# mmurooka/SMPLpp

Hardware: NVIDIA B200
Metric: SMPL FK+LBS meshes/s (higher is better)
Workload: dtype f32

## Files before the change

### smplpp_b200/csrc/common.cuh

```cuda
#pragma once
#include <cuda_runtime.h>

#include <atomic>
#include <cstdint>
#include <cstdio>
#include <string>
#include <vector>

#include "../../include/smplpp_b200.h"

namespace sb
{
constexpr int kJoints = SMPLPP_JOINT_NUM;
constexpr int kShapeDim = SMPLPP_SHAPE_DIM;
constexpr int kPoseDim = SMPLPP_POSE_DIM;
constexpr int kBlendK = 224;
constexpr int kBlendKUsed = kPoseDim + kShapeDim + 1;
constexpr int kXformFloats = 12;
constexpr int kGroupVerts = 4;
constexpr int kGroupJoints = 8;

extern thread_local std::string g_last_error;
extern std::atomic<uint64_t> g_launch_count;

int fail(int code, const char * module, const std::string & msg);

#define SB_CUDA(expr)                                                                                   \
  do                                                                                                    \
  {                                                                                                     \
    cudaError_t err__ = (expr);                                                                         \
    if(err__ != cudaSuccess)                                                                            \
      return ::sb::fail(SMPLPP_ERR_CUDA, "CUDA", std::string(#expr) + ": " + cudaGetErrorString(err__)); \
  } while(0)

#define SB_LAUNCHED()                                                              \
  do                                                                               \
  {                                                                                \
    ::sb::g_launch_count.fetch_add(1, std::memory_order_relaxed);                  \
    cudaError_t err__ = cudaPeekAtLastError();                                     \
    if(err__ != cudaSuccess)                                                       \
      return ::sb::fail(SMPLPP_ERR_CUDA, "CUDA", std::string("kernel launch: ") + cudaGetErrorString(err__)); \
  } while(0)

inline cudaStream_t as_stream(void * s)
{
  return static_cast<cudaStream_t>(s);
}

template<typename T>
inline T * align_up_ptr(void * p, size_t a = 256)
{
  return reinterpret_cast<T *>((reinterpret_cast<uintptr_t>(p) + a - 1) / a * a);
}

inline size_t align_up(size_t n, size_t a = 256)
{
  return (n + a - 1) / a * a;
}

inline bool first_call_on_device(bool (&done)[64])
{
  int dev = 0;
  if(cudaGetDevice(&dev) != cudaSuccess || dev < 0 || dev >= 64) return true;
  if(done[dev]) return false;
  done[dev] = true;
  return true;
}

struct ModelDev
{
  int V = 0;
  int Vpad = 0;
  int F = 0;
  int kmax = 0;
  float * basis = nullptr;
  uint8_t * lbs_joint = nullptr;
  float * lbs_weight = nullptr;
  float * lbs_wsum = nullptr;
  int8_t * group_nj = nullptr;
  uint8_t * group_joint = nullptr;
  float * group_w = nullptr;
  float * joint_template = nullptr;
  float * joint_shape = nullptr;
  int parent[kJoints];
  int depth[kJoints];
  int max_depth = 0;
  int32_t * faces = nullptr;
  int32_t * adj_offset = nullptr;
  int32_t * adj_faces = nullptr;
  float * weights_dense = nullptr;
  uint32_t * vert_jmask = nullptr;
  void * basis_split[2] = {nullptr, nullptr};
  alignas(64) unsigned char tmapA[2][128] = {};
  int tc_tiles = 0;
  bool tc_ready = false;
  void * basis_f16 = nullptr;
  alignas(64) unsigned char tmapA16[128] = {};
  int tc2_basis_exp = 0;
  int tc2_tiles = 0;
  bool tc2_ready = false;
  void * basis_img16 = nullptr;
  bool tc3_ready = false;
  int sm_count = 0;
};
}

struct smplpp_model
{
  sb::ModelDev d;
  std::vector<int32_t> h_faces;
  std::vector<int32_t> h_adj_offset;
  std::vector<int32_t> h_adj_faces;
  std::vector<float> h_basis;
  std::vector<float> h_weights;
  std::vector<uint32_t> h_vert_jmask;
  std::vector<float> h_joint_template, h_joint_shape;
  struct HostPipe
  {
    cudaStream_t compute = nullptr, copy = nullptr;
    cudaEvent_t done[2] = {nullptr, nullptr};
    cudaEvent_t drained[2] = {nullptr, nullptr};
    void * dev_in = nullptr;
    size_t dev_in_bytes = 0;
    void * dev_out[2] = {nullptr, nullptr};
    size_t dev_out_bytes = 0;
    void * dev_joints = nullptr;
    size_t dev_joints_bytes = 0;
    void * ws = nullptr;
    size_t ws_bytes = 0;
    void * pin_in = nullptr;
    size_t pin_in_bytes = 0;
    void * pin_out[2] = {nullptr, nullptr};
    size_t pin_out_bytes = 0;
  } pipe;
};
```

### smplpp_b200/csrc/forward.cu

```cuda
#include "common.cuh"
#include "forward.cuh"
#include "ik2.cuh"
#include "ik_poseblend.cuh"
#include "ik_solve.cuh"
#include "tc3_layout.cuh"
#include "vposer.cuh"

using namespace sb;

namespace sb
{
std::atomic<int> g_forward_variant{0};
std::atomic<int> g_lbs_variant{2};
}


__device__ __forceinline__ void rodrigues3(float x, float y, float z, float * R)
{
  const float eps = 1e-8f;
  float ax = x + eps, ay = y + eps, az = z + eps;
  float a = sqrtf(ax * ax + ay * ay + az * az);
  float ux = x / a, uy = y / a, uz = z / a;
  float s, c;
  sincosf(a, &s, &c);
  float oc = 1.f - c;
  R[0] = 1.f + oc * (-(uz * uz) - uy * uy);
  R[1] = s * (-uz) + oc * (uy * ux);
  R[2] = s * uy + oc * (uz * ux);
  R[3] = s * uz + oc * (ux * uy);
  R[4] = 1.f + oc * (-(uz * uz) - ux * ux);
  R[5] = s * (-ux) + oc * (uz * uy);
  R[6] = s * (-uy) + oc * (ux * uz);
  R[7] = s * ux + oc * (uy * uz);
  R[8] = 1.f + oc * (-(uy * uy) - ux * ux);
}

constexpr int kChainWarps = 8;

__global__ void __launch_bounds__(kChainWarps * 32)
    pose_chain_kernel(ChainTopo topo, const float * __restrict__ joint_template,
                      const float * __restrict__ joint_shape, int B, const float * __restrict__ beta,
                      long long beta_stride, const float * __restrict__ theta, float * __restrict__ coef,
                      float * __restrict__ xforms, float * __restrict__ joints_out, float * __restrict__ xforms44_out,
                      uint8_t * __restrict__ img_b, uint8_t * __restrict__ img_g, int Bpad)
{
  __shared__ float sG[kChainWarps][kJoints][12];
  __shared__ float sJ[kChainWarps][kJoints][3];
  __shared__ float sC[kChainWarps][kBlendK];
  const int warp = threadIdx.x >> 5, lane = threadIdx.x & 31;
  const long long b = static_cast<long long>(blockIdx.x) * kChainWarps + warp;
  if(b >= B)
  {
    if(img_b && b < Bpad)
    {
      const long long fb = b / tc3::NF;
      const int nf = static_cast<int>(b - fb * tc3::NF);
      const uint4 z = make_uint4(0u, 0u, 0u, 0u);
      if(lane < tc3::KP / 8)
      {
        uint8_t * blk = img_b + (static_cast<size_t>(fb) * tc3::NKB + lane / 4) * (2 * tc3::B_PART);
        const uint32_t o = static_cast<uint32_t>(tc3::coef_row(nf) * tc3::ROWB + (lane % 4) * 16);
        *reinterpret_cast<uint4 *>(blk + tc3::swz64(o)) = z;
        *reinterpret_cast<uint4 *>(blk + tc3::swz64(tc3::B_PART + o)) = z;
      }
      uint8_t * blk = img_g + (static_cast<size_t>(fb) * tc3::NSUB + nf / tc3::SUBF) * tc3::G_STAGE;
      for(int c = lane; c < kXformFloats * 4; c += 32)
      {
        const uint32_t o = static_cast<uint32_t>(((nf % tc3::SUBF) * kXformFloats + c / 4) * tc3::ROWB + (c % 4) * 16);
        *reinterpret_cast<uint4 *>(blk + tc3::swz64(o)) = z;
        *reinterpret_cast<uint4 *>(blk + tc3::swz64(tc3::G_PART + o)) = z;
      }
    }
    return;
  }

  const float * bp = beta + b * beta_stride;
  float R[9], Jt[3] = {0.f, 0.f, 0.f}, t[3];
  if(lane < kJoints)
  {
    const float * th = theta + (b * (kJoints + 1) + 1 + lane) * 3;
    rodrigues3(th[0], th[1], th[2], R);
#pragma unroll
    for(int k = 0; k < 3; k++)
    {
      float acc = joint_template[lane * 3 + k];
#pragma unroll
      for(int i = 0; i < kShapeDim; i++) acc = fmaf(joint_shape[(lane * 3 + k) * kShapeDim + i], bp[i], acc);
      Jt[k] = acc;
      sJ[warp][lane][k] = acc;
    }
  }
  __syncwarp();
  const int parent = lane < kJoints ? topo.parent[lane] : -1;
  const int depth = lane < kJoints ? topo.depth[lane] : -1;
  if(lane < kJoints)
  {
#pragma unroll
    for(int k = 0; k < 3; k++) t[k] = parent >= 0 ? Jt[k] - sJ[warp][parent][k] : Jt[k];
  }
  float G[12];
  for(int d = 0; d <= topo.max_depth; d++)
  {
    if(depth == d)
    {
      if(parent < 0)
      {
#pragma unroll
        for(int r = 0; r < 3; r++)
        {
          G[4 * r + 0] = R[3 * r + 0];
          G[4 * r + 1] = R[3 * r + 1];
          G[4 * r + 2] = R[3 * r + 2];
          G[4 * r + 3] = t[r];
        }
      }
      else
      {
        const float * P = sG[warp][parent];
#pragma unroll
        for(int r = 0; r < 3; r++)
        {
          float p0 = P[4 * r + 0], p1 = P[4 * r + 1], p2 = P[4 * r + 2], p3 = P[4 * r + 3];
#pragma unroll
          for(int c = 0; c < 3; c++) G[4 * r + c] = p0 * R[c] + p1 * R[3 + c] + p2 * R[6 + c];
          G[4 * r + 3] = p0 * t[0] + p1 * t[1] + p2 * t[2] + p3;
        }
      }
#pragma unroll
      for(int e = 0; e < 12; e++) sG[warp][lane][e] = G[e];
    }
    __syncwarp();
  }
  if(lane < kJoints)
  {
#pragma unroll
    for(int r = 0; r < 3; r++) G[4 * r + 3] -= G[4 * r + 0] * Jt[0] + G[4 * r + 1] * Jt[1] + G[4 * r + 2] * Jt[2];
    if(xforms)
    {
      float4 * dst = reinterpret_cast<float4 *>(xforms + (b * kJoints + lane) * 12);
      dst[0] = make_float4(G[0], G[1], G[2], G[3]);
      dst[1] = make_float4(G[4], G[5], G[6], G[7]);
      dst[2] = make_float4(G[8], G[9], G[10], G[11]);
    }
    if(xforms44_out)
    {
      float4 * dst = reinterpret_cast<float4 *>(xforms44_out + (b * kJoints + lane) * 16);
      dst[0] = make_float4(G[0], G[1], G[2], G[3]);
      dst[1] = make_float4(G[4], G[5], G[6], G[7]);
      dst[2] = make_float4(G[8], G[9], G[10], G[11]);
      dst[3] = make_float4(0.f, 0.f, 0.f, 1.f);
    }
    if(joints_out)
    {
#pragma unroll
      for(int k = 0; k < 3; k++) joints_out[(b * kJoints + lane) * 3 + k] = Jt[k];
    }
  }
  if(img_g)
  {
    __syncwarp();
    if(lane < kJoints)
    {
#pragma unroll
      for(int e = 0; e < 12; e++) sG[warp][lane][e] = G[e];
    }
    __syncwarp();
    const long long fb = b / tc3::NF;
    const int nf = static_cast<int>(b - fb * tc3::NF);
    uint8_t * blk = img_g + (static_cast<size_t>(fb) * tc3::NSUB + nf / tc3::SUBF) * tc3::G_STAGE;
    for(int c = lane; c < kXformFloats * 4; c += 32)
    {
      const int e = c / 4, cj = c % 4;
      float x[8];
#pragma unroll
      for(int jj = 0; jj < 8; jj++)
      {
        const int j = cj * 8 + jj;
        x[jj] = j < kJoints ? sG[warp][j][e] * static_cast<float>(1 << tc3::G_EXP) : 0.f;
      }
      const uint32_t o = static_cast<uint32_t>(((nf % tc3::SUBF) * kXformFloats + e) * tc3::ROWB + cj * 16);
      tc3::split8_store(x, blk + tc3::swz64(o), blk + tc3::swz64(tc3::G_PART + o));
    }
  }
  if(coef)
  {
    if(lane >= 1 && lane < kJoints)
    {
#pragma unroll
      for(int e = 0; e < 9; e++) sC[warp][9 * (lane - 1) + e] = R[e] - ((e == 0 || e == 4 || e == 8) ? 1.f : 0.f);
    }
    if(lane < kShapeDim) sC[warp][kPoseDim + lane] = bp[lane];
    if(lane >= kShapeDim && lane < kShapeDim + 1 + (kBlendK - kBlendKUsed))
      sC[warp][kPoseDim + lane] = lane == kShapeDim ? 1.f : 0.f;
    __syncwarp();
    for(int i = lane; i < kBlendK; i += 32) coef[b * kBlendK + i] = sC[warp][i];
    if(img_b && lane < tc3::KP / 8)
    {
      float x[8];
#pragma unroll
      for(int e = 0; e < 8; e++) x[e] = lane * 8 + e < tc3::KUSED ? sC[warp][lane * 8 + e] * static_cast<float>(1 << tc3::COEF_EXP) : 0.f;
      const long long fb = b / tc3::NF;
      const int r = tc3::coef_row(static_cast<int>(b - fb * tc3::NF));
      uint8_t * blk = img_b + (static_cast<size_t>(fb) * tc3::NKB + lane / 4) * (2 * tc3::B_PART);
      const uint32_t o = static_cast<uint32_t>(r * tc3::ROWB + (lane % 4) * 16);
      tc3::split8_store(x, blk + tc3::swz64(o), blk + tc3::swz64(tc3::B_PART + o));
    }
  }
}

namespace k2
{
constexpr int BM = 64, BNV = 64, BN = BNV * 3, BK = 16, THREADS = 256;
constexpr int TM = 4, TNV = 4, TN = TNV * 3;
constexpr int AS_LD = BM + 4, BS_LD = BN + 4;
constexpr int GS_LD = kJoints * 12;
constexpr size_t SMEM_AB = sizeof(float) * 2 * BK * (AS_LD + BS_LD);
constexpr size_t SMEM_G = sizeof(float) * BM * GS_LD;
constexpr size_t SMEM_TOTAL = SMEM_AB + SMEM_G;
}

__device__ __forceinline__ void cp_async16(void * smem, const void * gmem)
{
  unsigned s = static_cast<unsigned>(__cvta_generic_to_shared(smem));
  asm volatile("cp.async.cg.shared.global [%0], [%1], 16;\n" ::"r"(s), "l"(gmem));
}
__device__ __forceinline__ void cp_async_commit()
{
  asm volatile("cp.async.commit_group;\n" ::);
}
__device__ __forceinline__ void cp_async_wait_all()
{
  asm volatile("cp.async.wait_all;\n" ::);
}

template<bool kSkin>
__global__ void __launch_bounds__(k2::THREADS, 2)
    blend_skin_ffma_kernel(const float * __restrict__ basis, const uint8_t * __restrict__ lbs_joint,
                           const float * __restrict__ lbs_weight, const float * __restrict__ lbs_wsum, int V, int Vpad,
                           int kmax, int B, const float * __restrict__ coef, const float * __restrict__ xforms,
                           const float * __restrict__ theta, float * __restrict__ out)
{
  using namespace k2;
  extern __shared__ __align__(16) float smem[];
  float * As = smem;
  float * Bs = smem + 2 * BK * AS_LD;
  float * Gs = smem + 2 * BK * (AS_LD + BS_LD);

  const int tid = threadIdx.x;
  const int tx = tid & 15, ty = tid >> 4;
  const int v0 = blockIdx.x * BNV;
  const int m0 = blockIdx.y * BM;

  if(kSkin)
  {
    for(int i = tid; i < BM * GS_LD / 4; i += THREADS)
    {
      int row = i / (GS_LD / 4), q = i % (GS_LD / 4);
      int b = min(m0 + row, B - 1);
      cp_async16(Gs + row * GS_LD + q * 4, xforms + static_cast<size_t>(b) * GS_LD + q * 4);
    }
    cp_async_commit();
  }

  const int a_row = tid >> 2, a_q = tid & 3;
  const float * a_src = coef + static_cast<size_t>(min(m0 + a_row, B - 1)) * kBlendK + a_q * 4;
  const float * b_src[3];
  int b_row[3], b_q[3];
#pragma unroll
  for(int i = 0; i < 3; i++)
  {
    int idx = tid + i * THREADS;
    b_row[i] = idx >> 2;
    b_q[i] = idx & 3;
    b_src[i] = basis + (static_cast<size_t>(v0) * 3 + b_row[i]) * kBlendK + b_q[i] * 4;
  }
  float4 a_reg, b_reg[3];
  auto load_chunk = [&](int kc) {
    a_reg = __ldg(reinterpret_cast<const float4 *>(a_src + kc * BK));
#pragma unroll
    for(int i = 0; i < 3; i++) b_reg[i] = __ldg(reinterpret_cast<const float4 *>(b_src[i] + kc * BK));
  };
  auto store_chunk = [&](int buf) {
    float * as = As + buf * BK * AS_LD + (a_q * 4) * AS_LD + a_row;
    as[0] = a_reg.x;
    as[AS_LD] = a_reg.y;
    as[2 * AS_LD] = a_reg.z;
    as[3 * AS_LD] = a_reg.w;
#pragma unroll
    for(int i = 0; i < 3; i++)
    {
      float * bs = Bs + buf * BK * BS_LD + (b_q[i] * 4) * BS_LD + b_row[i];
      bs[0] = b_reg[i].x;
      bs[BS_LD] = b_reg[i].y;
      bs[2 * BS_LD] = b_reg[i].z;
      bs[3 * BS_LD] = b_reg[i].w;
    }
  };

  float acc[TM][TN];
#pragma unroll
  for(int i = 0; i < TM; i++)
#pragma unroll
    for(int j = 0; j < TN; j++) acc[i][j] = 0.f;

  constexpr int NK = kBlendK / BK;
  load_chunk(0);
  store_chunk(0);
  __syncthreads();
  for(int kc = 0; kc < NK; kc++)
  {
    const int buf = kc & 1;
    if(kc + 1 < NK) load_chunk(kc + 1);
    const float * as = As + buf * BK * AS_LD + ty * TM;
    const float * bs = Bs + buf * BK * BS_LD + tx * TN;
#pragma unroll
    for(int k = 0; k < BK; k++)
    {
      float4 a4 = *reinterpret_cast<const float4 *>(as + k * AS_LD);
      float4 b0 = *reinterpret_cast<const float4 *>(bs + k * BS_LD);
      float4 b1 = *reinterpret_cast<const float4 *>(bs + k * BS_LD + 4);
      float4 b2 = *reinterpret_cast<const float4 *>(bs + k * BS_LD + 8);
      float a[TM] = {a4.x, a4.y, a4.z, a4.w};
      float bb[TN] = {b0.x, b0.y, b0.z, b0.w, b1.x, b1.y, b1.z, b1.w, b2.x, b2.y, b2.z, b2.w};
#pragma unroll
      for(int i = 0; i < TM; i++)
#pragma unroll
        for(int j = 0; j < TN; j++) acc[i][j] = fmaf(a[i], bb[j], acc[i][j]);
    }
    if(kc + 1 < NK)
    {
      store_chunk(buf ^ 1);
      __syncthreads();
    }
  }

  const int vbase = v0 + tx * TNV;
  const bool vec_ok = (V & 1) == 0;
  if(kSkin)
  {
    cp_async_wait_all();
    __syncthreads();
    uint8_t jn[TNV][4];
    float jw[TNV][4], inv_ws[TNV];
    if(kmax <= 4)
    {
#pragma unroll
      for(int jv = 0; jv < TNV; jv++)
      {
#pragma unroll
        for(int k = 0; k < 4; k++)
        {
          bool on = k < kmax;
          jn[jv][k] = on ? lbs_joint[static_cast<size_t>(k) * Vpad + vbase + jv] : 0;
          jw[jv][k] = on ? lbs_weight[static_cast<size_t>(k) * Vpad + vbase + jv] : 0.f;
        }
        inv_ws[jv] = 1.f / lbs_wsum[vbase + jv];
      }
    }
#pragma unroll
    for(int i = 0; i < TM; i++)
    {
      const int b = m0 + ty * TM + i;
      if(b >= B) continue;
      const float * g = Gs + (ty * TM + i) * GS_LD;
      const float * tr = theta + static_cast<size_t>(b) * (kJoints + 1) * 3;
      const float trx = tr[0], try_ = tr[1], trz = tr[2];
      float o[TN];
#pragma unroll
      for(int jv = 0; jv < TNV; jv++)
      {
        const float rx = acc[i][3 * jv], ry = acc[i][3 * jv + 1], rz = acc[i][3 * jv + 2];
        float ox = 0.f, oy = 0.f, oz = 0.f, iw;
        if(kmax <= 4)
        {
#pragma unroll
          for(int k = 0; k < 4; k++)
          {
            const float4 * gj = reinterpret_cast<const float4 *>(g + jn[jv][k] * 12);
            float4 r0 = gj[0], r1 = gj[1], r2 = gj[2];
            float w = jw[jv][k];
            ox = fmaf(w, fmaf(r0.x, rx, fmaf(r0.y, ry, fmaf(r0.z, rz, r0.w))), ox);
            oy = fmaf(w, fmaf(r1.x, rx, fmaf(r1.y, ry, fmaf(r1.z, rz, r1.w))), oy);
            oz = fmaf(w, fmaf(r2.x, rx, fmaf(r2.y, ry, fmaf(r2.z, rz, r2.w))), oz);
          }
          iw = inv_ws[jv];
        }
        else
        {
          const int v = vbase + jv;
          for(int k = 0; k < kmax; k++)
          {
            const float4 * gj = reinterpret_cast<const float4 *>(g + lbs_joint[static_cast<size_t>(k) * Vpad + v] * 12);
            float4 r0 = gj[0], r1 = gj[1], r2 = gj[2];
            float w = lbs_weight[static_cast<size_t>(k) * Vpad + v];
            ox = fmaf(w, fmaf(r0.x, rx, fmaf(r0.y, ry, fmaf(r0.z, rz, r0.w))), ox);
            oy = fmaf(w, fmaf(r1.x, rx, fmaf(r1.y, ry, fmaf(r1.z, rz, r1.w))), oy);
            oz = fmaf(w, fmaf(r2.x, rx, fmaf(r2.y, ry, fmaf(r2.z, rz, r2.w))), oz);
          }
          iw = 1.f / lbs_wsum[v];
        }
        o[3 * jv] = fmaf(ox, iw, trx);
        o[3 * jv + 1] = fmaf(oy, iw, try_);
        o[3 * jv + 2] = fmaf(oz, iw, trz);
      }
      float * dst = out + (static_cast<size_t>(b) * V + vbase) * 3;
      if(vbase + TNV <= V && vec_ok)
      {
#pragma unroll
        for(int q = 0; q < TN / 2; q++) reinterpret_cast<float2 *>(dst)[q] = make_float2(o[2 * q], o[2 * q + 1]);
      }
      else
      {
        for(int q = 0; q < TN; q++)
          if(vbase + q / 3 < V) dst[q] = o[q];
      }
    }
  }
  else
  {
#pragma unroll
    for(int i = 0; i < TM; i++)
    {
      const int b = m0 + ty * TM + i;
      if(b >= B) continue;
      float * dst = out + (static_cast<size_t>(b) * V + vbase) * 3;
      if(vbase + TNV <= V && vec_ok)
      {
#pragma unroll
        for(int q = 0; q < TN / 2; q++) reinterpret_cast<float2 *>(dst)[q] = make_float2(acc[i][2 * q], acc[i][2 * q + 1]);
      }
      else
      {
        for(int q = 0; q < TN; q++)
          if(vbase + q / 3 < V) dst[q] = acc[i][q];
      }
    }
  }
}

namespace k3
{
constexpr int THREADS = 256, VPL = kGroupVerts, VPC = THREADS * VPL;
constexpr int FR = 16;
}

template<bool kAffine, bool kVec2>
__global__ void __launch_bounds__(k3::THREADS, 2)
    lbs_kernel(const uint8_t * __restrict__ lbs_joint, const float * __restrict__ lbs_weight,
               const float * __restrict__ lbs_wsum, const int8_t * __restrict__ group_nj,
               const uint8_t * __restrict__ group_joint, const float * __restrict__ group_w, int V, int Vpad, int kmax,
               int B, const float * __restrict__ rest, const float * __restrict__ xforms,
               const float * __restrict__ root, int root_stride, float * __restrict__ out)
{
  using namespace k3;
  constexpr int XF = kAffine ? 12 : 16;
  constexpr int XFP = kAffine ? 12 : 20;
  __shared__ __align__(16) float Gs[FR][kJoints * XFP];
  const int tid = threadIdx.x;
  const int b0 = blockIdx.y * FR;
  const int nfr = min(FR, B - b0);
  for(int i = tid; i < nfr * kJoints * XF / 4; i += THREADS)
  {
    const int fr = i / (kJoints * XF / 4), rem = i % (kJoints * XF / 4);
    const int j = rem / (XF / 4), q = rem % (XF / 4);
    *reinterpret_cast<float4 *>(&Gs[fr][j * XFP + 4 * q]) =
        __ldg(reinterpret_cast<const float4 *>(xforms + static_cast<size_t>(b0) * kJoints * XF) + i);
  }
  const int v = (blockIdx.x * THREADS + tid) * VPL;
  const int g = v / VPL;
  const int nvalid = min(VPL, V - v);
  int nj = -1;
  float gw[kGroupJoints][VPL], iw[VPL];
  unsigned gj_lo = 0, gj_hi = 0;
  if(nvalid > 0)
  {
    nj = group_nj ? group_nj[g] : -1;
#pragma unroll
    for(int u = 0; u < VPL; u++) iw[u] = 1.f / lbs_wsum[min(v + u, V - 1)];
    if(nj >= 0)
    {
      const uint2 jj = __ldg(reinterpret_cast<const uint2 *>(group_joint + static_cast<size_t>(g) * kGroupJoints));
      gj_lo = jj.x, gj_hi = jj.y;
#pragma unroll
      for(int k = 0; k < kGroupJoints; k++)
      {
        const float4 w = __ldg(reinterpret_cast<const float4 *>(group_w + (static_cast<size_t>(g) * kGroupJoints + k) * VPL));
        gw[k][0] = w.x, gw[k][1] = w.y, gw[k][2] = w.z, gw[k][3] = w.w;
      }
    }
  }
  __syncthreads();
  if(nvalid <= 0) return;
  const bool full = nvalid == VPL;
  float rn[3 * VPL];
  auto load_frame = [&](int f) {
    const size_t base = (static_cast<size_t>(b0 + f) * V + v) * 3;
    if(kVec2 && full)
    {
      const float2 * src = reinterpret_cast<const float2 *>(rest + base);
#pragma unroll
      for(int q = 0; q < 6; q++)
      {
        const float2 t = __ldcs(src + q);
        rn[2 * q] = t.x, rn[2 * q + 1] = t.y;
      }
    }
    else
    {
#pragma unroll
      for(int q = 0; q < 3 * VPL; q++) rn[q] = q < 3 * nvalid ? rest[base + q] : 0.f;
    }
  };
  load_frame(0);
  for(int f = 0; f < nfr; f++)
  {
    const size_t base = (static_cast<size_t>(b0 + f) * V + v) * 3;
    float r[3 * VPL];
#pragma unroll
    for(int q = 0; q < 3 * VPL; q++) r[q] = rn[q];
    if(f + 1 < nfr) load_frame(f + 1);
    float tx = 0.f, ty = 0.f, tz = 0.f;
    if(root)
    {
      const float * rp = root + static_cast<size_t>(b0 + f) * root_stride;
      tx = rp[0], ty = rp[1], tz = rp[2];
    }
    float o[3 * VPL], ow[VPL];
#pragma unroll
    for(int q = 0; q < 3 * VPL; q++) o[q] = 0.f;
#pragma unroll
    for(int u = 0; u < VPL; u++) ow[u] = 0.f;
    if(nj >= 0)
    {
#pragma unroll
      for(int k = 0; k < kGroupJoints; k++)
      {
        if(k < nj)
        {
          const int j = ((k < 4 ? gj_lo : gj_hi) >> (8 * (k & 3))) & 0xff;
          const float4 * gjp = reinterpret_cast<const float4 *>(&Gs[f][j * XFP]);
          const float4 r0 = gjp[0], r1 = gjp[1], r2 = gjp[2];
          float4 r3 = make_float4(0.f, 0.f, 0.f, 1.f);
          if(!kAffine) r3 = gjp[3];
#pragma unroll
          for(int u = 0; u < VPL; u++)
          {
            const float w = gw[k][u];
            const float rx = r[3 * u], ry = r[3 * u + 1], rz = r[3 * u + 2];
            o[3 * u] = fmaf(w, fmaf(r0.x, rx, fmaf(r0.y, ry, fmaf(r0.z, rz, r0.w))), o[3 * u]);
            o[3 * u + 1] = fmaf(w, fmaf(r1.x, rx, fmaf(r1.y, ry, fmaf(r1.z, rz, r1.w))), o[3 * u + 1]);
            o[3 * u + 2] = fmaf(w, fmaf(r2.x, rx, fmaf(r2.y, ry, fmaf(r2.z, rz, r2.w))), o[3 * u + 2]);
            if(!kAffine) ow[u] = fmaf(w, fmaf(r3.x, rx, fmaf(r3.y, ry, fmaf(r3.z, rz, r3.w))), ow[u]);
          }
        }
      }
    }
    else
    {
      for(int u = 0; u < nvalid; u++)
      {
        const float rx = r[3 * u], ry = r[3 * u + 1], rz = r[3 * u + 2];
        float ox = 0.f, oy = 0.f, oz = 0.f, o4 = 0.f;
        for(int k = 0; k < kmax; k++)
        {
          const float w = lbs_weight[static_cast<size_t>(k) * Vpad + v + u];
          const float4 * gjp = reinterpret_cast<const float4 *>(&Gs[f][lbs_joint[static_cast<size_t>(k) * Vpad + v + u] * XFP]);
          const float4 r0 = gjp[0], r1 = gjp[1], r2 = gjp[2];
          ox = fmaf(w, fmaf(r0.x, rx, fmaf(r0.y, ry, fmaf(r0.z, rz, r0.w))), ox);
          oy = fmaf(w, fmaf(r1.x, rx, fmaf(r1.y, ry, fmaf(r1.z, rz, r1.w))), oy);
          oz = fmaf(w, fmaf(r2.x, rx, fmaf(r2.y, ry, fmaf(r2.z, rz, r2.w))), oz);
          if(!kAffine)
          {
            const float4 r3 = gjp[3];
            o4 = fmaf(w, fmaf(r3.x, rx, fmaf(r3.y, ry, fmaf(r3.z, rz, r3.w))), o4);
          }
        }
#pragma unroll
        for(int uu = 0; uu < VPL; uu++)
          if(uu == u) o[3 * uu] = ox, o[3 * uu + 1] = oy, o[3 * uu + 2] = oz, ow[uu] = o4;
      }
    }
#pragma unroll
    for(int u = 0; u < VPL; u++)
    {
      const float inv = kAffine ? iw[u] : 1.f / ow[u];
      o[3 * u] = fmaf(o[3 * u], inv, tx);
      o[3 * u + 1] = fmaf(o[3 * u + 1], inv, ty);
      o[3 * u + 2] = fmaf(o[3 * u + 2], inv, tz);
    }
    if(kVec2 && full)
    {
      float2 * dst = reinterpret_cast<float2 *>(out + base);
#pragma unroll
      for(int q = 0; q < 6; q++) __stcs(dst + q, make_float2(o[2 * q], o[2 * q + 1]));
    }
    else
    {
#pragma unroll
      for(int q = 0; q < 3 * VPL; q++)
        if(q < 3 * nvalid) out[base + q] = o[q];
    }
  }
}

__global__ void rodrigues_kernel(long long n, const float * __restrict__ theta, float * __restrict__ rot)
{
  long long i = static_cast<long long>(blockIdx.x) * blockDim.x + threadIdx.x;
  if(i >= n) return;
  float R[9];
  rodrigues3(theta[3 * i], theta[3 * i + 1], theta[3 * i + 2], R);
#pragma unroll
  for(int e = 0; e < 9; e++) rot[9 * i + e] = R[e];
}

__global__ void blend_generic_kernel(int B, int V, const float * __restrict__ beta, const float * __restrict__ rot,
                                     const float * __restrict__ shape_basis, const float * __restrict__ pose_basis,
                                     float * __restrict__ shape_bs, float * __restrict__ pose_bs)
{
  long long i = static_cast<long long>(blockIdx.x) * blockDim.x + threadIdx.x;
  if(i >= static_cast<long long>(B) * V * 3) return;
  int b = static_cast<int>(i / (static_cast<long long>(V) * 3));
  long long vk = i % (static_cast<long long>(V) * 3);
  const float * pb = pose_basis + vk * kPoseDim;
  const float * r = rot + static_cast<size_t>(b) * kJoints * 9 + 9;
  float acc = 0.f;
  for(int d = 0; d < kPoseDim; d++)
  {
    int e = d % 9;
    float c = r[d] - ((e == 0 || e == 4 || e == 8) ? 1.f : 0.f);
    acc = fmaf(c, pb[d], acc);
  }
  pose_bs[i] = acc;
  const float * sb_ = shape_basis + vk * kShapeDim;
  float s = 0.f;
  for(int d = 0; d < kShapeDim; d++) s = fmaf(beta[b * kShapeDim + d], sb_[d], s);
  shape_bs[i] = s;
}

__global__ void linear_combine_kernel(long long n, long long vk_count, const float * __restrict__ templ,
                                      const float * __restrict__ shape_bs, const float * __restrict__ pose_bs,
                                      float * __restrict__ rest)
{
  long long i = static_cast<long long>(blockIdx.x) * blockDim.x + threadIdx.x;
  if(i >= n) return;
  rest[i] = templ[i % vk_count] + shape_bs[i] + pose_bs[i];
}

__global__ void joint_regress_kernel(int B, int V, const float * __restrict__ templ, const float * __restrict__ jreg,
                                     const float * __restrict__ shape_bs, float * __restrict__ joints)
{
  int w = (blockIdx.x * blockDim.x + threadIdx.x) >> 5, lane = threadIdx.x & 31;
  if(w >= B * kJoints * 3) return;
  int b = w / (kJoints * 3), j = (w / 3) % kJoints, k = w % 3;
  float acc = 0.f;
  for(int v = lane; v < V; v += 32)
    acc = fmaf(jreg[static_cast<size_t>(j) * V + v], templ[3 * v + k] + shape_bs[(static_cast<size_t>(b) * V + v) * 3 + k], acc);
#pragma unroll
  for(int o = 16; o > 0; o >>= 1) acc += __shfl_xor_sync(0xffffffffu, acc, o);
  if(lane == 0) joints[w] = acc;
}

__global__ void world_transform_kernel(int B, const long long * __restrict__ kine_tree, const float * __restrict__ joints,
                                       const float * __restrict__ rot, float * __restrict__ out)
{
  int b = blockIdx.x * blockDim.x + threadIdx.x;
  if(b >= B) return;
  float G[kJoints][12];
  const float * J = joints + static_cast<size_t>(b) * kJoints * 3;
  const float * R = rot + static_cast<size_t>(b) * kJoints * 9;
  for(int j = 0; j < kJoints; j++)
  {
    long long p = kine_tree[j];
    const float * Rj = R + 9 * j;
    if(j == 0 || p < 0 || p >= kJoints)
    {
      for(int r = 0; r < 3; r++)
      {
        for(int c = 0; c < 3; c++) G[j][4 * r + c] = Rj[3 * r + c];
        G[j][4 * r + 3] = J[3 * j + r];
      }
    }
    else
    {
      float t[3] = {J[3 * j] - J[3 * p], J[3 * j + 1] - J[3 * p + 1], J[3 * j + 2] - J[3 * p + 2]};
      for(int r = 0; r < 3; r++)
      {
        float p0 = G[p][4 * r], p1 = G[p][4 * r + 1], p2 = G[p][4 * r + 2], p3 = G[p][4 * r + 3];
        for(int c = 0; c < 3; c++) G[j][4 * r + c] = p0 * Rj[c] + p1 * Rj[3 + c] + p2 * Rj[6 + c];
        G[j][4 * r + 3] = p0 * t[0] + p1 * t[1] + p2 * t[2] + p3;
      }
    }
  }
  float * o = out + static_cast<size_t>(b) * kJoints * 16;
  for(int j = 0; j < kJoints; j++)
  {
    for(int r = 0; r < 3; r++)
    {
      for(int c = 0; c < 3; c++) o[16 * j + 4 * r + c] = G[j][4 * r + c];
      o[16 * j + 4 * r + 3] =
          G[j][4 * r + 3] - (G[j][4 * r] * J[3 * j] + G[j][4 * r + 1] * J[3 * j + 1] + G[j][4 * r + 2] * J[3 * j + 2]);
    }
    o[16 * j + 12] = 0.f, o[16 * j + 13] = 0.f, o[16 * j + 14] = 0.f, o[16 * j + 15] = 1.f;
  }
}

__global__ void lbs_dense_kernel(int B, int V, const float * __restrict__ weights, const float * __restrict__ rest,
                                 const float * __restrict__ xf, const float * __restrict__ root,
                                 float * __restrict__ out)
{
  long long i = static_cast<long long>(blockIdx.x) * blockDim.x + threadIdx.x;
  if(i >= static_cast<long long>(B) * V) return;
  int b = static_cast<int>(i / V), v = static_cast<int>(i % V);
  float rx = rest[3 * i], ry = rest[3 * i + 1], rz = rest[3 * i + 2];
  float M[16];
  for(int e = 0; e < 16; e++) M[e] = 0.f;
  for(int j = 0; j < kJoints; j++)
  {
    float w = weights[static_cast<size_t>(v) * kJoints + j];
    const float * g = xf + (static_cast<size_t>(b) * kJoints + j) * 16;
    for(int e = 0; e < 16; e++) M[e] = fmaf(w, g[e], M[e]);
  }
  float h[4];
  for(int r = 0; r < 4; r++) h[r] = M[4 * r] * rx + M[4 * r + 1] * ry + M[4 * r + 2] * rz + M[4 * r + 3];
  for(int k = 0; k < 3; k++) out[3 * i + k] = h[k] / h[3] + (root ? root[3 * b + k] : 0.f);
}

__device__ __forceinline__ void normalize3(float & x, float & y, float & z)
{
  float n = fmaxf(sqrtf(x * x + y * y + z * z), 1e-12f);
  x /= n, y /= n, z /= n;
}

__device__ __forceinline__ void face_normal(const float * __restrict__ verts, const int32_t * __restrict__ faces, int f,
                                            float & nx, float & ny, float & nz)
{
  const float * a = verts + 3 * faces[3 * f], *b = verts + 3 * faces[3 * f + 1], *c = verts + 3 * faces[3 * f + 2];
  float e1x = b[0] - a[0], e1y = b[1] - a[1], e1z = b[2] - a[2];
  float e2x = c[0] - a[0], e2y = c[1] - a[1], e2z = c[2] - a[2];
  nx = e1y * e2z - e1z * e2y;
  ny = e1z * e2x - e1x * e2z;
  nz = e1x * e2y - e1y * e2x;
  normalize3(nx, ny, nz);
}

__global__ void normals_kernel(const int32_t * __restrict__ faces, const int32_t * __restrict__ adj_offset,
                               const int32_t * __restrict__ adj_faces, int V, int F, int B,
                               const float * __restrict__ verts, int nF, const long long * __restrict__ face_idx,
                               float * __restrict__ fn, int nV, const long long * __restrict__ vert_idx,
                               float * __restrict__ vn)
{
  long long i = static_cast<long long>(blockIdx.x) * blockDim.x + threadIdx.x;
  const int per = nF + nV;
  if(i >= static_cast<long long>(B) * per) return;
  int b = static_cast<int>(i / per), it = static_cast<int>(i % per);
  const float * vb = verts + static_cast<size_t>(b) * V * 3;
  if(it < nF)
  {
    long long f = face_idx[it];
    float x = 0.f, y = 0.f, z = 0.f;
    if(f >= 0 && f < F) face_normal(vb, faces, static_cast<int>(f), x, y, z);
    float * o = fn + (static_cast<size_t>(b) * nF + it) * 3;
    o[0] = x, o[1] = y, o[2] = z;
  }
  else
  {
    it -= nF;
    long long v = vert_idx[it];
    float ax = 0.f, ay = 0.f, az = 0.f;
    if(v >= 0 && v < V)
    {
      int s = adj_offset[v], e = adj_offset[v + 1];
      float w = 1.f / static_cast<float>(e - s);
      for(int k = s; k < e; k++)
      {
        float x, y, z;
        face_normal(vb, faces, adj_faces[k], x, y, z);
        ax = fmaf(w, x, ax), ay = fmaf(w, y, ay), az = fmaf(w, z, az);
      }
      normalize3(ax, ay, az);
    }
    float * o = vn + (static_cast<size_t>(b) * nV + it) * 3;
    o[0] = ax, o[1] = ay, o[2] = az;
  }
}

namespace sb
{
ChainTopo make_topo(const ModelDev & d)
{
  ChainTopo t;
  for(int j = 0; j < kJoints; j++)
  {
    t.parent[j] = d.parent[j];
    t.depth[j] = d.depth[j];
  }
  t.max_depth = d.max_depth;
  return t;
}

int launch_pose_chain(const ModelDev & d, cudaStream_t st, int B, const float * beta, long long beta_stride,
                      const float * theta, float * coef, float * xforms, float * joints, float * xforms44,
                      void * tc3_scratch)
{
  const int Bpad = tc3_scratch ? static_cast<int>(align_up(static_cast<size_t>(B), tc3::NF)) : B;
  uint8_t * img_b = static_cast<uint8_t *>(tc3_scratch);
  uint8_t * img_g = tc3_scratch ? img_b + tc3::img_g_offset(Bpad) : nullptr;
  int grid = (Bpad + kChainWarps - 1) / kChainWarps;
  pose_chain_kernel<<<grid, kChainWarps * 32, 0, st>>>(make_topo(d), d.joint_template, d.joint_shape, B, beta,
                                                       beta_stride, theta, coef, xforms, joints, xforms44, img_b, img_g, Bpad);
  SB_LAUNCHED();
  return SMPLPP_OK;
}

int launch_blend_skin_ffma(const ModelDev & d, cudaStream_t st, int B, const float * coef, const float * xforms,
                           const float * theta, float * out, bool skin)
{
  static bool configured[64] = {};
  if(first_call_on_device(configured))
  {
    SB_CUDA(cudaFuncSetAttribute(blend_skin_ffma_kernel<true>, cudaFuncAttributeMaxDynamicSharedMemorySize,
                                 static_cast<int>(k2::SMEM_TOTAL)));
    SB_CUDA(cudaFuncSetAttribute(blend_skin_ffma_kernel<false>, cudaFuncAttributeMaxDynamicSharedMemorySize,
                                 static_cast<int>(k2::SMEM_AB)));
  }
  dim3 grid(d.Vpad / k2::BNV, (B + k2::BM - 1) / k2::BM);
  if(skin)
    blend_skin_ffma_kernel<true><<<grid, k2::THREADS, k2::SMEM_TOTAL, st>>>(
        d.basis, d.lbs_joint, d.lbs_weight, d.lbs_wsum, d.V, d.Vpad, d.kmax, B, coef, xforms, theta, out);
  else
    blend_skin_ffma_kernel<false><<<grid, k2::THREADS, k2::SMEM_AB, st>>>(
        d.basis, d.lbs_joint, d.lbs_weight, d.lbs_wsum, d.V, d.Vpad, d.kmax, B, coef, xforms, theta, out);
  SB_LAUNCHED();
  return SMPLPP_OK;
}

int launch_lbs(const ModelDev & d, cudaStream_t st, int B, const float * rest, const float * xforms, bool affine,
               const float * root, int root_stride, float * out)
{
  if(affine && g_lbs_variant == 2 && lbs_tc_usable(d, rest, out, xforms))
    return launch_lbs_tc(d, st, B, rest, xforms, kXformFloats, root, root_stride, out);
  if(affine && g_lbs_variant == 0 && lbs_tma_usable(d, rest, out, xforms))
    return launch_lbs_tma(d, st, B, rest, xforms, root, root_stride, out);
  dim3 grid((d.V + k3::VPC - 1) / k3::VPC, (B + k3::FR - 1) / k3::FR);
  const bool vec2 = (d.V & 1) == 0 && (reinterpret_cast<uintptr_t>(rest) & 7) == 0 && (reinterpret_cast<uintptr_t>(out) & 7) == 0;
#define SB_LBS(AFF, VEC)                                                                                               \
  lbs_kernel<AFF, VEC><<<grid, k3::THREADS, 0, st>>>(d.lbs_joint, d.lbs_weight, d.lbs_wsum, d.group_nj, d.group_joint, \
                                                     d.group_w, d.V, d.Vpad, d.kmax, B, rest, xforms, root,           \
                                                     root_stride, out)
  if(affine && vec2)
    SB_LBS(true, true);
  else if(affine)
    SB_LBS(true, false);
  else if(vec2)
    SB_LBS(false, true);
  else
    SB_LBS(false, false);
#undef SB_LBS
  SB_LAUNCHED();
  return SMPLPP_OK;
}
}

extern "C" int smplpp_set_forward_variant(int variant)
{
  if(variant == 100 || variant == 101)
  {
    g_tc_grid_order = variant - 100;
    return SMPLPP_OK;
  }
  if(variant == 300 || variant == 301)
  {
    g_vposer_jac_variant = variant - 300;
    return SMPLPP_OK;
  }
  if(variant >= 200 && variant <= 202)
  {
    g_lbs_variant = variant - 200;
    return SMPLPP_OK;
  }
  if(variant >= 400 && variant <= 402)
  {
    g_ik_variant = variant - 400;
    return SMPLPP_OK;
  }
  if(variant == 410 || variant == 411)
  {
    g_solve_variant = variant - 410;
    return SMPLPP_OK;
  }
  if(variant >= 420 && variant <= 422)
  {
    g_poseblend_variant = variant - 420;
    return SMPLPP_OK;
  }
  if(variant < 0 || variant > 6) return fail(SMPLPP_ERR_INVALID, "SMPL", "unknown forward variant");
  g_forward_variant = variant;
  return SMPLPP_OK;
}

extern "C" size_t smplpp_forward_workspace_bytes(const smplpp_model_t * model, int64_t batch)
{
  if(!model || batch < 1) return 0;
  size_t bpad = align_up(static_cast<size_t>(batch), 128);
  size_t bytes = 512;
  bytes += align_up(bpad * kBlendK * sizeof(float));
  bytes += align_up(bpad * kJoints * 12 * sizeof(float));
  bytes += tc_coef_split_bytes(batch);
  bytes += std::max(tc2_frame_operand_bytes(batch), tc3_frame_operand_bytes(batch));
  bytes += align_up(static_cast<size_t>(batch) * model->d.V * 3 * sizeof(float));
  return bytes;
}

extern "C" int smplpp_forward(const smplpp_model_t * model, void * stream, int64_t batch, const float * beta,
                              int64_t beta_stride, const float * theta, float * vertices, float * joints,
                              float * transforms, float * rest_shape, void * workspace, size_t workspace_bytes)
{
  if(!model || batch < 1 || !beta || !theta) return fail(SMPLPP_ERR_INVALID, "SMPL", "Cannot launch a SMPL model!");
  if(batch > (1ll << 24)) return fail(SMPLPP_ERR_INVALID, "SMPL", "Cannot launch a SMPL model! (batch too large)");
  if(!workspace || workspace_bytes < smplpp_forward_workspace_bytes(model, batch))
    return fail(SMPLPP_ERR_INVALID, "SMPL", "Cannot launch a SMPL model! (workspace too small)");
  const ModelDev & d = model->d;
  const int B = static_cast<int>(batch);
  cudaStream_t st = as_stream(stream);
  size_t bpad = align_up(static_cast<size_t>(batch), 128);
  char * ws = align_up_ptr<char>(workspace);
  float * coef = reinterpret_cast<float *>(ws);
  ws += align_up(bpad * kBlendK * sizeof(float));
  float * xforms = reinterpret_cast<float *>(ws);
  ws += align_up(bpad * kJoints * 12 * sizeof(float));
  void * coef_split = ws;
  ws += tc_coef_split_bytes(batch);
  void * tc2_scratch = ws;
  ws += std::max(tc2_frame_operand_bytes(batch), tc3_frame_operand_bytes(batch));
  float * rest_ws = reinterpret_cast<float *>(ws);

  const bool need_verts = vertices != nullptr;
  const bool need_rest = rest_shape != nullptr;
  int variant = g_forward_variant;
  if(variant == 0) variant = model->d.tc3_ready ? 6 : (model->d.tc2_ready ? 5 : (model->d.tc_ready ? 2 : 1));
  if(((variant == 2 || variant == 4) && !model->d.tc_ready) || (variant == 5 && !model->d.tc2_ready)
     || (variant == 6 && !model->d.tc3_ready))
    return fail(SMPLPP_ERR_INVALID, "SMPL", "tcgen05 blend variant is not available for this model");
  const bool fused_images = variant == 6 && need_verts && !need_rest;
  int rc = launch_pose_chain(d, st, B, beta, beta_stride, theta, (need_verts || need_rest) ? coef : nullptr, xforms,
                             joints, transforms, fused_images ? tc2_scratch : nullptr);
  if(rc != SMPLPP_OK) return rc;
  if(need_rest || (need_verts && variant == 3))
  {
    float * rest = need_rest ? rest_shape : rest_ws;
    rc = launch_blend_skin_ffma(d, st, B, coef, xforms, theta, rest, false);
    if(rc != SMPLPP_OK) return rc;
    if(need_verts) rc = launch_lbs(d, st, B, rest, xforms, true, theta, (kJoints + 1) * 3, vertices);
    return rc;
  }
  if(need_verts)
  {
    if(variant == 6)
      rc = launch_blend_skin_tc3(d, st, B, coef, xforms, tc2_scratch, theta, vertices, true);
    else if(variant == 5)
      rc = launch_blend_skin_tc2(d, st, B, coef, xforms, tc2_scratch, theta, vertices);
    else if(variant == 2 || variant == 4)
      rc = launch_blend_skin_tc(d, st, B, coef, coef_split, xforms, theta, vertices, variant == 2);
    else
      rc = launch_blend_skin_ffma(d, st, B, coef, xforms, theta, vertices, true);
  }
  return rc;
}


extern "C" int smplpp_blend_shape(void * stream, int64_t batch, int64_t V, const float * beta, const float * theta,
                                  const float * shape_basis, const float * pose_basis, float * shape_bs, float * pose_bs,
                                  float * pose_rot)
{
  if(batch < 1 || V < 1 || !beta) return fail(SMPLPP_ERR_INVALID, "BlendShape", "Failed to set beta!");
  if(!theta) return fail(SMPLPP_ERR_INVALID, "BlendShape", "Failed to set theta!");
  if(!shape_basis || !pose_basis || !shape_bs || !pose_bs || !pose_rot)
    return fail(SMPLPP_ERR_INVALID, "BlendShape", "Cannot blend pose-dependented shape!");
  cudaStream_t st = as_stream(stream);
  long long n = batch * kJoints;
  rodrigues_kernel<<<static_cast<unsigned>((n + 127) / 128), 128, 0, st>>>(n, theta, pose_rot);
  SB_LAUNCHED();
  long long total = batch * V * 3;
  blend_generic_kernel<<<static_cast<unsigned>((total + 127) / 128), 128, 0, st>>>(
      static_cast<int>(batch), static_cast<int>(V), beta, pose_rot, shape_basis, pose_basis, shape_bs, pose_bs);
  SB_LAUNCHED();
  return SMPLPP_OK;
}

extern "C" int smplpp_joint_regression(void * stream, int64_t batch, int64_t V, const float * templ, const float * jreg,
                                       const float * shape_bs, const float * pose_bs, float * rest, float * joints)
{
  if(batch < 1 || V < 1 || !templ || !shape_bs || !pose_bs || !rest)
    return fail(SMPLPP_ERR_INVALID, "JointRegression", "Cannot linearly combine shapes!");
  if(!jreg || !joints) return fail(SMPLPP_ERR_INVALID, "JointRegression", "Cannot regress vertices to joints!");
  cudaStream_t st = as_stream(stream);
  long long n = batch * V * 3;
  linear_combine_kernel<<<static_cast<unsigned>((n + 255) / 256), 256, 0, st>>>(n, V * 3, templ, shape_bs, pose_bs, rest);
  SB_LAUNCHED();
  long long warps = batch * kJoints * 3;
  joint_regress_kernel<<<static_cast<unsigned>((warps * 32 + 127) / 128), 128, 0, st>>>(
      static_cast<int>(batch), static_cast<int>(V), templ, jreg, shape_bs, joints);
  SB_LAUNCHED();
  return SMPLPP_OK;
}

extern "C" int smplpp_world_transformation(void * stream, int64_t batch, const int64_t * kine_tree, const float * joints,
                                           const float * pose_rot, float * transforms)
{
  if(batch < 1 || !kine_tree || !joints || !pose_rot || !transforms)
    return fail(SMPLPP_ERR_INVALID, "WorldTransformation", "Cannot transform bones locally!");
  world_transform_kernel<<<static_cast<unsigned>((batch + 63) / 64), 64, 0, as_stream(stream)>>>(
      static_cast<int>(batch), reinterpret_cast<const long long *>(kine_tree), joints, pose_rot, transforms);
  SB_LAUNCHED();
  return SMPLPP_OK;
}

extern "C" int smplpp_linear_blend_skinning(void * stream, int64_t batch, int64_t V, const float * weights,
                                            const float * rest, const float * transforms, const float * root_pos,
                                            float * vertices)
{
  if(batch < 1 || V < 1 || !weights) return fail(SMPLPP_ERR_INVALID, "LinearBlendSkinning", "Failed to set weights!");
  if(!rest || !transforms || !vertices)
    return fail(SMPLPP_ERR_INVALID, "LinearBlendSkinning", "Cannot convert Cartesian coordinates to homogeneous one!");
  long long n = batch * V;
  lbs_dense_kernel<<<static_cast<unsigned>((n + 127) / 128), 128, 0, as_stream(stream)>>>(
      static_cast<int>(batch), static_cast<int>(V), weights, rest, transforms, root_pos, vertices);
  SB_LAUNCHED();
  return SMPLPP_OK;
}

extern "C" int smplpp_model_skinning(const smplpp_model_t * model, void * stream, int64_t batch, const float * rest,
                                     const float * transforms, const float * root_pos, float * vertices)
{
  if(!model || batch < 1 || !rest || !transforms || !vertices)
    return fail(SMPLPP_ERR_INVALID, "LinearBlendSkinning", "Failed to get vertices of new pose!");
  return launch_lbs(model->d, as_stream(stream), static_cast<int>(batch), rest, transforms, false, root_pos, 3, vertices);
}

extern "C" int smplpp_normals(const smplpp_model_t * model, void * stream, int64_t batch, const float * vertices,
                              int64_t n_faces, const int64_t * face_idx, float * face_normals, int64_t n_verts,
                              const int64_t * vert_idx, float * vertex_normals)
{
  if(!model || batch < 1 || !vertices || n_faces < 0 || n_verts < 0 || (n_faces > 0 && (!face_idx || !face_normals))
     || (n_verts > 0 && (!vert_idx || !vertex_normals)))
    return fail(SMPLPP_ERR_INVALID, "SMPL", "Failed to get face indices!");
  long long total = batch * (n_faces + n_verts);
  if(total == 0) return SMPLPP_OK;
  const ModelDev & d = model->d;
  normals_kernel<<<static_cast<unsigned>((total + 127) / 128), 128, 0, as_stream(stream)>>>(
      d.faces, d.adj_offset, d.adj_faces, d.V, d.F, static_cast<int>(batch), vertices, static_cast<int>(n_faces),
      reinterpret_cast<const long long *>(face_idx), face_normals, static_cast<int>(n_verts),
      reinterpret_cast<const long long *>(vert_idx), vertex_normals);
  SB_LAUNCHED();
  return SMPLPP_OK;
}

extern "C" int smplpp_model_skinning34(const smplpp_model_t * model, void * stream, int64_t batch, const float * rest,
                                       const float * transforms34, const float * root_pos, float * vertices)
{
  if(!model || batch < 1 || !rest || !transforms34 || !vertices)
    return fail(SMPLPP_ERR_INVALID, "LinearBlendSkinning", "Failed to get vertices of new pose!");
  return launch_lbs(model->d, as_stream(stream), static_cast<int>(batch), rest, transforms34, true, root_pos, 3, vertices);
}
```

### smplpp_b200/csrc/skin_tc3.cu

```cuda
#include <cuda.h>
#include <cuda_fp16.h>

#include <cstdio>
#include <cstdlib>
#include <vector>

#include "forward.cuh"
#include "skin_common.cuh"
#include "tc3_layout.cuh"
#include "tc_ptx.cuh"

using namespace sb;

namespace tc3
{
struct Params
{
  int V, B, Bpad, ntiles, nfb, nitems;
  float scale_p, scale_m;
  const uint8_t * img_a;
  const uint8_t * img_b;
  const uint8_t * img_g;
  const float * basis;
  const float * weights;
  const float * wsum;
  const float * theta;
  float * out;
  long long * dbg;
  int dbg_mode;
};

}

__global__ void basis_image_f16_kernel(const float * __restrict__ basis, int V, int ntiles, float scale, uint8_t * __restrict__ img)
{
  const long long i = static_cast<long long>(blockIdx.x) * blockDim.x + threadIdx.x;
  const long long n = static_cast<long long>(ntiles) * 3 * tc3::MV * tc3::KP;
  if(i >= n) return;
  const int k = static_cast<int>(i % tc3::KP);
  const long long row = i / tc3::KP;
  const int r = static_cast<int>(row % tc3::MV);
  const int plane = static_cast<int>((row / tc3::MV) % 3);
  const int tile = static_cast<int>(row / (3 * tc3::MV));
  const int v = tile * tc3::MV + r;
  const float x = (v < V && k < tc3::KUSED) ? basis[(static_cast<size_t>(3) * v + plane) * kBlendK + k] * scale : 0.f;
  const __half hi = __float2half_rn(x);
  const __half lo = __float2half_rn(x - __half2float(hi));
  uint8_t * blk = img + (static_cast<size_t>(tile) * tc3::NKB + k / 32) * (2 * tc3::A_PART);
  const uint32_t o = static_cast<uint32_t>(plane * tc3::MV * tc3::ROWB + r * tc3::ROWB + (k % 32) * 2);
  *reinterpret_cast<__half *>(blk + tc3::swz64(o)) = hi;
  *reinterpret_cast<__half *>(blk + tc3::swz64(tc3::A_PART + o)) = lo;
}

__global__ void frame_images3_kernel(const float * __restrict__ coef, const float * __restrict__ xforms, int B, int Bpad,
                                     uint8_t * __restrict__ img_b, uint8_t * __restrict__ img_g)
{
  const long long i = static_cast<long long>(blockIdx.x) * blockDim.x + threadIdx.x;
  constexpr int CK = tc3::KP / 8;
  constexpr int CJ = tc3::KJ / 8;
  const long long n_coef = static_cast<long long>(Bpad) * CK;
  const long long n_xf = static_cast<long long>(Bpad) * kXformFloats * CJ;
  float x[8];
  if(i < n_coef)
  {
    const int ck = static_cast<int>(i % CK);
    const long long f = i / CK;
    if(f < B)
    {
      const float4 a = __ldg(reinterpret_cast<const float4 *>(coef + f * tc3::KP + ck * 8));
      const float4 b = __ldg(reinterpret_cast<const float4 *>(coef + f * tc3::KP + ck * 8 + 4));
      x[0] = a.x, x[1] = a.y, x[2] = a.z, x[3] = a.w, x[4] = b.x, x[5] = b.y, x[6] = b.z, x[7] = b.w;
    }
#pragma unroll
    for(int e = 0; e < 8; e++) x[e] = (f < B && ck * 8 + e < tc3::KUSED) ? x[e] * static_cast<float>(1 << tc3::COEF_EXP) : 0.f;
    const long long fb = f / tc3::NF;
    const int r = tc3::coef_row(static_cast<int>(f - fb * tc3::NF));
    uint8_t * blk = img_b + (static_cast<size_t>(fb) * tc3::NKB + ck / 4) * (2 * tc3::B_PART);
    const uint32_t o = static_cast<uint32_t>(r * tc3::ROWB + (ck % 4) * 16);
    tc3::split8_store(x, blk + tc3::swz64(o), blk + tc3::swz64(tc3::B_PART + o));
  }
  else if(i < n_coef + n_xf)
  {
    const long long q = i - n_coef;
    const int cj = static_cast<int>(q % CJ);
    const long long row = q / CJ;
    const int e = static_cast<int>(row % kXformFloats);
    const long long f = row / kXformFloats;
#pragma unroll
    for(int jj = 0; jj < 8; jj++)
    {
      const int j = cj * 8 + jj;
      x[jj] = (f < B && j < kJoints) ? __ldg(xforms + (f * kJoints + j) * kXformFloats + e) * static_cast<float>(1 << tc3::G_EXP) : 0.f;
    }
    const long long fb = f / tc3::NF;
    const int nf = static_cast<int>(f - fb * tc3::NF);
    uint8_t * blk = img_g + (static_cast<size_t>(fb) * tc3::NSUB + nf / tc3::SUBF) * tc3::G_STAGE;
    const uint32_t o = static_cast<uint32_t>(((nf % tc3::SUBF) * kXformFloats + e) * tc3::ROWB + cj * 16);
    tc3::split8_store(x, blk + tc3::swz64(o), blk + tc3::swz64(tc3::G_PART + o));
  }
}

template<int STAGES, int GSLOTS, int EPI, bool DBG = false>
__global__ void __launch_bounds__(tc3::THREADS, 1)
    blend_skin_tc3_kernel(const tc3::Params p)
{
  using namespace tc3;
  using L = Layout<STAGES, GSLOTS, EPI>;
  constexpr int OFF_G = L::OFF_G, OFF_STG = L::OFF_STG, OFF_BAR = L::OFF_BAR;
  extern __shared__ uint8_t smem_raw[];
  uint8_t * smem = reinterpret_cast<uint8_t *>((reinterpret_cast<uintptr_t>(smem_raw) + 1023) & ~uintptr_t(1023));
  uint64_t * bars = reinterpret_cast<uint64_t *>(smem + OFF_BAR);
  const uint32_t smem32 = (ptx::smem_u32(smem_raw) + 1023u) & ~1023u;
  const uint32_t bar32 = smem32 + OFF_BAR;
  uint64_t * full = bars;
  uint64_t * empty = full + STAGES;
  uint64_t * g_full = empty + STAGES;
  uint64_t * g_empty = g_full + GSLOTS;
  uint64_t * m_full = g_empty + GSLOTS;
  uint64_t * m_empty = m_full + 2;
  uint64_t * p_full = m_empty + 2;
  uint64_t * rest_free = p_full + 1;
  uint64_t * w_ready = rest_free + 1;
  uint32_t * tmem_slot = reinterpret_cast<uint32_t *>(w_ready + 1);

  const int warp = threadIdx.x >> 5, lane = threadIdx.x & 31;
  const int it0 = static_cast<int>(static_cast<long long>(blockIdx.x) * p.nitems / gridDim.x);
  const int it1 = static_cast<int>(static_cast<long long>(blockIdx.x + 1) * p.nitems / gridDim.x);
  const int nit = it1 - it0;

  if(warp == 0 && lane == 0)
  {
    for(int s = 0; s < STAGES; s++)
    {
      ptx::mbar_init(&full[s], 1);
      ptx::mbar_init(&empty[s], 1);
    }
    for(int s = 0; s < GSLOTS; s++)
    {
      ptx::mbar_init(&g_full[s], 1);
      ptx::mbar_init(&g_empty[s], 1);
    }
    for(int i = 0; i < 2; i++)
    {
      ptx::mbar_init(&m_full[i], 1);
      ptx::mbar_init(&m_empty[i], EPI_WARPS);
    }
    ptx::mbar_init(p_full, 1);
    ptx::mbar_init(rest_free, EPI_WARPS);
    ptx::mbar_init(w_ready, 4);
    ptx::fence_barrier_init();
  }
  if(warp == 1) ptx::tmem_alloc<TMEM_COLS>(tmem_slot);
  ptx::tc_fence_before();
  __syncthreads();
  ptx::tc_fence_after();
  const uint32_t tmem_base = *tmem_slot;
  long long * dbg = (DBG && p.dbg) ? p.dbg + static_cast<size_t>(blockIdx.x) * 256 : nullptr;
  long long w_stage = 0, w_gfull = 0, w_mempty = 0, w_rest = 0, w_pfull = 0, w_mfull = 0;
#define TC3_OFF(bit) (DBG && (p.dbg_mode & (bit)))
#define TC3_TIMED(acc, stmt) do { if constexpr(DBG) { const long long t_ = clock64(); stmt; acc += clock64() - t_; } else { stmt; } } while(0)

  if(warp < CTRL_WARPS)
  {
  asm volatile("setmaxnreg.dec.sync.aligned.u32 32;");
  if(warp == 0)
  {
    if(ptx::elect_one())
    {
      const int total_kb = TC3_OFF(32) ? 0 : nit * NKB;
      int kb = 0, tile = it0 / p.nfb, fb = it0 % p.nfb;
      for(int kbn = 0; kbn < total_kb; kbn++)
      {
        const uint32_t s = static_cast<uint32_t>(kbn % STAGES);
        const uint8_t * srca = p.img_a + (static_cast<size_t>(tile) * NKB + kb) * (2 * A_PART);
        const uint8_t * srcb = p.img_b + (static_cast<size_t>(fb) * NKB + kb) * (2 * B_PART);
        const uint32_t dst = smem32 + s * STAGE, fbar = bar32 + 8 * s;
        ptx::mbar_wait_a(bar32 + 8 * (STAGES + s), ((kbn / STAGES) & 1) ^ 1);
        ptx::mbar_expect_tx_a(fbar, STAGE);
        ptx::bulk_load_1d_a(dst, srca, 2 * A_PART, fbar);
        ptx::bulk_load_1d_a(dst + 2 * A_PART, srcb, 2 * B_PART, fbar);
        if(dbg && kbn < 14) dbg[34 + kbn] = clock64();
        if(++kb == NKB)
        {
          kb = 0;
          if(++fb == p.nfb) fb = 0, tile++;
        }
      }
    }
  }
  else if(warp == 2)
  {
    if(ptx::elect_one())
    {
      const int total_g = TC3_OFF(64) ? 0 : nit * NSUB;
      int sb = 0, fb = it0 % p.nfb;
      for(int gn = 0; gn < total_g; gn++)
      {
        const uint32_t s = static_cast<uint32_t>(gn % GSLOTS);
        const uint8_t * src = p.img_g + (static_cast<size_t>(fb) * NSUB + sb) * G_STAGE;
        const uint32_t fbar = bar32 + 8 * (2 * STAGES + s);
        ptx::mbar_wait_a(bar32 + 8 * (2 * STAGES + GSLOTS + s), ((gn / GSLOTS) & 1) ^ 1);
        ptx::mbar_expect_tx_a(fbar, G_STAGE);
        ptx::bulk_load_1d_a(smem32 + OFF_G + s * G_STAGE, src, G_STAGE, fbar);
        if(++sb == NSUB)
        {
          sb = 0;
          if(++fb == p.nfb) fb = 0;
        }
      }
    }
  }
  else if(warp == 1 || warp == 3)
  {
    if(ptx::elect_one())
    {
      constexpr uint32_t idesc1 = ptx::make_idesc_f16(MV, NF);
      constexpr uint32_t idesc2 = ptx::make_idesc_f16(MV, SUBN);
      static_assert(NSUB % GSLOTS == 0 && ((NSUB / GSLOTS) & 1) == 0, "transform ring: slot and parity of a sub-batch do not depend on the item");
      static_assert((NSUB & 3) == 0, "matrix buffers: parity of a sub-batch does not depend on the item");
      constexpr uint32_t DHI = ptx::smem_desc_hi<ROWB>();
      const uint32_t smem16 = smem32 >> 4;
      const uint32_t a_full = bar32;
      const uint32_t a_empty = a_full + 8 * STAGES, a_gfull = a_empty + 8 * STAGES, a_gempty = a_gfull + 8 * GSLOTS,
                     a_mfull = a_gempty + 8 * GSLOTS, a_mempty = a_mfull + 16, a_pfull = a_mempty + 16, a_rest = a_pfull + 8,
                     a_wready = a_rest + 8;
      auto g1_mma = [&](uint32_t st16, int hpar, int i, uint32_t acc) {
        const int t = i / 3, c = i % 3;
        const int a_part = hpar == 0 ? (t == 2 ? 1 : 0) : (t == 0 ? 1 : 0);
        const int b_part = hpar == 0 ? 0 : (t == 0 ? 0 : 1);
        const int ks = hpar == 0 ? (t == 1 ? 1 : 0) : (t == 1 ? 0 : 1);
        ptx::umma_f16_ss_lo(tmem_base + c * NF, st16 + ((a_part * A_PART + c * MV * ROWB + ks * 32) >> 4),
                            st16 + ((2 * A_PART + b_part * B_PART + ks * 32) >> 4), DHI, idesc1, acc);
      };
      auto g2_mma = [&](uint32_t dm, uint32_t aw, uint32_t sg16, int j) {
        const int prod = j >> 1, ks = j & 1;
        const int pa = prod == 1 ? 1 : 0, pb = prod == 2 ? 1 : 0;
        ptx::umma_f16_ts_lo(dm, aw + pa * (KJ / 2) + ks * 8, sg16 + ((pb * G_PART + ks * 32) >> 4), DHI, idesc2, j != 0 ? 1u : 0u);
      };
      auto g1_half = [&](int h, int kbn0) {
        const int kbn = kbn0 + (h >> 1);
        const uint32_t s = static_cast<uint32_t>(kbn % STAGES);
        const uint32_t st16 = smem16 + s * (STAGE >> 4);
        if((h & 1) == 0)
        {
          if(!TC3_OFF(32)) TC3_TIMED(w_stage, ptx::mbar_wait_a(a_full + 8 * s, (kbn / STAGES) & 1));
          ptx::tc_fence_after();
          if(dbg && kbn < 14) dbg[48 + kbn] = clock64();
#pragma unroll
          for(int i = 0; i < 9; i++)
            if(!DBG || !(p.dbg_mode & 8)) g1_mma(st16, 0, i, (h == 0 && i < 3) ? 0u : 1u);
        }
        else
        {
#pragma unroll
          for(int i = 0; i < 9; i++)
            if(!DBG || !(p.dbg_mode & 8)) g1_mma(st16, 1, i, 1u);
          if(!TC3_OFF(32)) ptx::tc_commit_a(a_empty + 8 * s);
        }
      };
      if(dbg) dbg[0] = clock64();
      if(nit > 0 && warp == 3)
      {
#pragma unroll
        for(int h = 0; h < 2 * NKB; h++) g1_half(h, 0);
        if(!TC3_OFF(512)) ptx::tc_commit_a(a_pfull);
      }
      if(dbg) dbg[1] = clock64();
      if(warp == 3)
      {
        for(int k = 0; k + 1 < nit; k++)
        {
          if(!TC3_OFF(512)) TC3_TIMED(w_rest, ptx::mbar_wait_a(a_rest, k & 1));
          ptx::tc_fence_after();
#pragma unroll
          for(int h = 0; h < 2 * NKB; h++) g1_half(h, (k + 1) * NKB);
          if(!TC3_OFF(512)) ptx::tc_commit_a(a_pfull);
        }
        if(dbg) dbg[64] = w_stage, dbg[67] = w_rest, dbg[69] = clock64();
      }
      int wcount = 0, prev_tile = -1;
      for(int k = 0; k < (warp == 3 ? 0 : nit); k++)
      {
        const int tile = (it0 + k) / p.nfb;
        if(tile != prev_tile)
        {
          ptx::mbar_wait_a(a_wready, wcount & 1);
          ptx::tc_fence_after();
          wcount++;
          prev_tile = tile;
        }
        const uint32_t aw = tmem_base + COL_W;
#pragma unroll
        for(int sb = 0; sb < NSUB; sb++)
        {
          const int b = sb & 1, gs = sb % GSLOTS;
          if(!TC3_OFF(64)) TC3_TIMED(w_gfull, ptx::mbar_wait_a(a_gfull + 8 * gs, (sb / GSLOTS) & 1));
          if(!TC3_OFF(256)) TC3_TIMED(w_mempty, ptx::mbar_wait_a(a_mempty + 8 * b, ((sb >> 1) & 1) ^ 1));
          ptx::tc_fence_after();
          const uint32_t sg16 = smem16 + ((OFF_G + gs * G_STAGE) >> 4);
          const uint32_t dm = tmem_base + COL_M + b * SUBN;
#pragma unroll
          for(int j = 0; j < 6; j++)
            if(!DBG || !(p.dbg_mode & 4)) g2_mma(dm, aw, sg16, j);
          if(!TC3_OFF(256)) ptx::tc_commit_a(a_mfull + 8 * b);
          if(!TC3_OFF(64)) ptx::tc_commit_a(a_gempty + 8 * gs);
        }
        if(dbg && k < 30) dbg[2 + k] = clock64();
      }
      if(dbg && warp == 1) dbg[65] = w_gfull, dbg[66] = w_mempty, dbg[68] = clock64();
    }
  }
  }
  else
  {
    asm volatile("setmaxnreg.inc.sync.aligned.u32 112;");
    const int ew = warp - CTRL_WARPS;
    const int q = warp & 3;
    const int fp = ew >> 2;
    const uint32_t lane_taddr = tmem_base + (static_cast<uint32_t>(q * 32) << 16);
    const uint32_t my_stg = ptx::smem_u32(smem + OFF_STG) + ew * STG_FLOATS * 4;
    const float sp = p.scale_p;
    const uint32_t a_mfull = bar32 + 16 * (STAGES + GSLOTS);
    const uint32_t a_mempty = a_mfull + 16, a_pfull = a_mempty + 16, a_rest = a_pfull + 8, a_wready = a_rest + 8;
    const unsigned fstride = static_cast<unsigned>(p.V) * 3u;
    int prev_tile = -1;
    int wv0 = 0, nvalid = 0;
    float T0 = 0.f, T1 = 0.f, T2 = 0.f, sm = 0.f;
    if(dbg && ew == 0 && lane == 0) dbg[32] = clock64();
    for(int k = 0; k < nit; k++)
    {
      const int item = it0 + k;
      const int tile = item / p.nfb, f0 = (item - tile * p.nfb) * NF;
      if(tile != prev_tile)
      {
        prev_tile = tile;
        wv0 = tile * MV + q * 32;
        const int vc = min(wv0 + lane, p.V - 1);
        nvalid = max(0, min(32, p.V - wv0));
        if(ew < 4)
        {
          skin::store_w_row_tmem(p.weights + static_cast<size_t>(vc) * kJoints, lane_taddr + COL_W);
          ptx::tmem_st_wait();
          ptx::tc_fence_before();
          __syncwarp();
          if(lane == 0) ptx::mbar_arrive_a(a_wready);
        }
        sm = p.scale_m / p.wsum[vc];
        const float * tp = p.basis + static_cast<size_t>(3) * vc * kBlendK + KUSED;
        T0 = __ldg(tp) * sm, T1 = __ldg(tp + kBlendK) * sm, T2 = __ldg(tp + 2 * kBlendK) * sm;
      }
      float trx = 0.f, try_ = 0.f, trz = 0.f;
      if(lane < FR_WARP)
      {
        const int f = min(f0 + (lane >> 1) * SUBF + fp * EPI_FR + (lane & 1), p.B - 1);
        const float * tq = p.theta + static_cast<size_t>(f) * ((kJoints + 1) * 3);
        trx = __ldg(tq), try_ = __ldg(tq + 1), trz = __ldg(tq + 2);
      }
      float R[3][FR_WARP];
      if(!TC3_OFF(512)) TC3_TIMED(w_pfull, ptx::mbar_wait_a(a_pfull, k & 1));
      ptx::tc_fence_after();
#pragma unroll
      for(int c = 0; c < 3; c++)
      {
        if(DBG && (p.dbg_mode & 16))
        {
#pragma unroll
          for(int i = 0; i < FR_WARP; i++) R[c][i] = 1.f;
          continue;
        }
        ptx::tmem_ld_x16(lane_taddr + c * NF + fp * FR_WARP, R[c]);
        ptx::tmem_ld_x8p(lane_taddr + c * NF + fp * FR_WARP + 16, R[c] + 16);
      }
      ptx::tmem_ld_wait();
      ptx::tc_fence_before();
      __syncwarp();
      if(lane == 0 && !TC3_OFF(512)) ptx::mbar_arrive_a(a_rest);
      {
        const float s = sp * sm;
#pragma unroll
        for(int i = 0; i < FR_WARP; i++)
        {
          R[0][i] = fmaf(R[0][i], s, T0);
          R[1][i] = fmaf(R[1][i], s, T1);
          R[2][i] = fmaf(R[2][i], s, T2);
        }
      }
      float * outp = p.out + (static_cast<size_t>(f0 + fp * EPI_FR) * p.V + wv0) * 3;
      float * outl = outp + lane * 3;
      const int nfv = lane < nvalid ? p.B - f0 - fp * EPI_FR : 0;
#pragma unroll
      for(int sb = 0; sb < NSUB; sb++)
      {
        const int h = sb & 1;
        float tr[EPI_FR][3];
#pragma unroll
        for(int t = 0; t < EPI_FR; t++)
        {
          tr[t][0] = __shfl_sync(0xffffffffu, trx, sb * EPI_FR + t);
          tr[t][1] = __shfl_sync(0xffffffffu, try_, sb * EPI_FR + t);
          tr[t][2] = __shfl_sync(0xffffffffu, trz, sb * EPI_FR + t);
        }
        if(!TC3_OFF(256)) TC3_TIMED(w_mfull, ptx::mbar_wait_a(a_mfull + 8 * h, (sb >> 1) & 1));
        ptx::tc_fence_after();
        float M[EPI_FR * kXformFloats];
        const uint32_t mcol = lane_taddr + COL_M + h * SUBN + fp * (EPI_FR * kXformFloats);
        if(DBG && (p.dbg_mode & 1))
        {
#pragma unroll
          for(int i = 0; i < EPI_FR * kXformFloats; i++) M[i] = 1.f + i;
        }
        else
        {
          ptx::tmem_ld_x16(mcol, M);
          ptx::tmem_ld_x8p(mcol + 16, M + 16);
        }
        ptx::tmem_ld_wait();
        ptx::tc_fence_before();
        __syncwarp();
        if(lane == 0 && !TC3_OFF(256)) ptx::mbar_arrive_a(a_mempty + 8 * h);
        if(TC3_OFF(128)) continue;
#pragma unroll
        for(int t = 0; t < EPI_FR; t++)
        {
          const float rx = R[0][sb * EPI_FR + t], ry = R[1][sb * EPI_FR + t], rz = R[2][sb * EPI_FR + t];
          const float * m = M + kXformFloats * t;
          const float ox = fmaf(m[0], rx, fmaf(m[1], ry, fmaf(m[2], rz, fmaf(m[3], sm, tr[t][0]))));
          const float oy = fmaf(m[4], rx, fmaf(m[5], ry, fmaf(m[6], rz, fmaf(m[7], sm, tr[t][1]))));
          const float oz = fmaf(m[8], rx, fmaf(m[9], ry, fmaf(m[10], rz, fmaf(m[11], sm, tr[t][2]))));
          if constexpr(EPI == 0)
          {
            const uint32_t sa = my_stg + (t * 96 + lane * 3) * 4;
            ptx::sts32(sa, ox);
            ptx::sts32(sa + 4, oy);
            ptx::sts32(sa + 8, oz);
          }
          else
          {
            float * o = outl + static_cast<size_t>((sb * SUBF + t) * fstride);
            if(sb * SUBF + t < nfv && (!DBG || !(p.dbg_mode & 2) || ox == 1.2345e30f))
            {
              __stcs(o, ox);
              __stcs(o + 1, oy);
              __stcs(o + 2, oz);
            }
          }
        }
        if constexpr(EPI != 0) continue;
        __syncwarp();
#pragma unroll
        for(int i = 0; i < EPI_FR * 48 / 32; i++)
        {
          const int idx = 32 * i + lane;
          const int t = idx / 48;
          const int w2 = idx - 48 * t;
          const int f = f0 + sb * SUBF + fp * EPI_FR + t;
          const float2 val = ptx::lds64(my_stg + idx * 8);
          if(f < p.B && 2 * w2 < 3 * nvalid)
            __stcs(reinterpret_cast<float2 *>(outp + (static_cast<size_t>(sb * SUBF + t) * p.V) * 3) + w2, val);
        }
        __syncwarp();
      }
    }
    if(dbg && (ew == 0 || ew == 15) && lane == 0)
    {
      if(ew == 0) dbg[33] = clock64();
      dbg[70 + (ew ? 2 : 0)] = w_pfull, dbg[71 + (ew ? 2 : 0)] = w_mfull;
    }
  }
#undef TC3_TIMED
#undef TC3_OFF
  ptx::tc_fence_before();
  __syncthreads();
  if(warp == 1) ptx::tmem_dealloc<TMEM_COLS>(tmem_base);
}

namespace sb
{
size_t tc3_frame_operand_bytes(int64_t batch)
{
  const size_t bpad = align_up(static_cast<size_t>(batch), tc3::NF);
  return align_up(2 * bpad * tc3::KP * sizeof(__half)) + align_up(2 * bpad * kXformFloats * tc3::KJ * sizeof(__half));
}

int tc3_prepare_model(ModelDev & d)
{
  d.tc3_ready = false;
  if(!d.tc2_ready) return SMPLPP_OK;
  const long long n = static_cast<long long>(d.tc2_tiles) * 3 * tc3::MV * tc3::KP;
  SB_CUDA(cudaMalloc(&d.basis_img16, static_cast<size_t>(2) * n * sizeof(__half)));
  basis_image_f16_kernel<<<static_cast<unsigned>((n + 255) / 256), 256>>>(d.basis, d.V, d.tc2_tiles, ldexpf(1.f, d.tc2_basis_exp),
                                                                         static_cast<uint8_t *>(d.basis_img16));
  SB_LAUNCHED();
  SB_CUDA(cudaDeviceSynchronize());
  SB_CUDA(cudaFuncSetAttribute(blend_skin_tc3_kernel<2, 6, 1>, cudaFuncAttributeMaxDynamicSharedMemorySize, tc3::Layout<2, 6, 1>::SMEM_BYTES));
  SB_CUDA(cudaFuncSetAttribute(blend_skin_tc3_kernel<2, 6, 1, true>, cudaFuncAttributeMaxDynamicSharedMemorySize, tc3::Layout<2, 6, 1>::SMEM_BYTES));
  SB_CUDA(cudaFuncSetAttribute(blend_skin_tc3_kernel<3, 3, 1>, cudaFuncAttributeMaxDynamicSharedMemorySize, tc3::Layout<3, 3, 1>::SMEM_BYTES));
  SB_CUDA(cudaFuncSetAttribute(blend_skin_tc3_kernel<2, 6, 0>, cudaFuncAttributeMaxDynamicSharedMemorySize, tc3::Layout<2, 6, 0>::SMEM_BYTES));
  int dev = 0;
  SB_CUDA(cudaGetDevice(&dev));
  SB_CUDA(cudaDeviceGetAttribute(&d.sm_count, cudaDevAttrMultiProcessorCount, dev));
  d.tc3_ready = d.sm_count > 0;
  return SMPLPP_OK;
}

void tc3_release_model(ModelDev & d)
{
  if(d.basis_img16) cudaFree(d.basis_img16);
  d.basis_img16 = nullptr;
  d.tc3_ready = false;
}

int launch_blend_skin_tc3(const ModelDev & d, cudaStream_t st, int B, const float * coef, const float * xforms, void * scratch,
                          const float * theta, float * out, bool images_ready)
{
  if(!d.tc3_ready) return fail(SMPLPP_ERR_INVALID, "SMPL", "pipelined tcgen05 skinning variant is not available for this model");
  if(reinterpret_cast<uintptr_t>(out) & 7) return fail(SMPLPP_ERR_INVALID, "SMPL", "tcgen05 variants need 8-byte aligned vertices");
  if(reinterpret_cast<uintptr_t>(scratch) & 127) return fail(SMPLPP_ERR_INVALID, "SMPL", "tcgen05 variants need a 128-byte aligned workspace");
  const int Bpad = static_cast<int>(align_up(static_cast<size_t>(B), tc3::NF));
  uint8_t * img_b = static_cast<uint8_t *>(scratch);
  uint8_t * img_g = img_b + tc3::img_g_offset(Bpad);
  if(!images_ready)
  {
    const long long n = static_cast<long long>(Bpad) * (tc3::KP + kXformFloats * tc3::KJ) / 8;
    frame_images3_kernel<<<static_cast<unsigned>((n + 255) / 256), 256, 0, st>>>(coef, xforms, B, Bpad, img_b, img_g);
    SB_LAUNCHED();
  }
  tc3::Params p;
  p.V = d.V;
  p.B = B;
  p.Bpad = Bpad;
  p.ntiles = d.tc2_tiles;
  p.nfb = Bpad / tc3::NF;
  p.nitems = p.ntiles * p.nfb;
  p.scale_p = ldexpf(1.f, -(d.tc2_basis_exp + tc3::COEF_EXP));
  p.scale_m = ldexpf(1.f, -(tc3::W_EXP + tc3::G_EXP));
  p.img_a = static_cast<const uint8_t *>(d.basis_img16);
  p.img_b = img_b;
  p.img_g = img_g;
  p.basis = d.basis;
  p.weights = d.weights_dense;
  p.wsum = d.lbs_wsum;
  p.theta = theta;
  p.out = out;
  int grid = p.nitems < d.sm_count ? p.nitems : d.sm_count;
  static const int grid_env = getenv("SMPLPP_TC3_GRID") ? atoi(getenv("SMPLPP_TC3_GRID")) : 0;
  static const int ring_env = getenv("SMPLPP_TC3_RING") ? atoi(getenv("SMPLPP_TC3_RING")) : 0;
  if(grid_env > 0 && grid_env < grid) grid = grid_env;
  static const bool dbg_on = getenv("SMPLPP_TC3_DBG") != nullptr;
  p.dbg = nullptr;
  p.dbg_mode = dbg_on ? atoi(getenv("SMPLPP_TC3_DBG")) >> 1 : 0;
  if(dbg_on)
  {
    SB_CUDA(cudaMalloc(&p.dbg, static_cast<size_t>(grid) * 256 * sizeof(long long)));
    SB_CUDA(cudaMemsetAsync(p.dbg, 0, static_cast<size_t>(grid) * 256 * sizeof(long long), st));
  }
  if(ring_env == 1)
    blend_skin_tc3_kernel<3, 3, 1><<<grid, tc3::THREADS, tc3::Layout<3, 3, 1>::SMEM_BYTES, st>>>(p);
  else if(ring_env == 2)
    blend_skin_tc3_kernel<2, 6, 0><<<grid, tc3::THREADS, tc3::Layout<2, 6, 0>::SMEM_BYTES, st>>>(p);
  else if(dbg_on)
    blend_skin_tc3_kernel<2, 6, 1, true><<<grid, tc3::THREADS, tc3::Layout<2, 6, 1>::SMEM_BYTES, st>>>(p);
  else
    blend_skin_tc3_kernel<2, 6, 1><<<grid, tc3::THREADS, tc3::Layout<2, 6, 1>::SMEM_BYTES, st>>>(p);
  SB_LAUNCHED();
  if(dbg_on)
  {
    SB_CUDA(cudaStreamSynchronize(st));
    std::vector<long long> h(static_cast<size_t>(grid) * 256);
    SB_CUDA(cudaMemcpy(h.data(), p.dbg, h.size() * sizeof(long long), cudaMemcpyDeviceToHost));
    cudaFree(p.dbg);
    for(int cta : {0, grid / 2})
    {
      const long long * t = h.data() + static_cast<size_t>(cta) * 256;
      fprintf(stderr, "[tc3 dbg] cta %d: first GEMM 1 issued +%lld | items", cta, t[1] - t[0]);
      for(int k = 0; k < 30 && t[2 + k]; k++) fprintf(stderr, " %lld", t[2 + k] - (k ? t[1 + k] : t[1]));
      fprintf(stderr, " | epilogue %lld .. %lld\n", t[32] - t[0], t[33] - t[0]);
      fprintf(stderr, "   stage loads issued (K-block 0..13):");
      for(int i = 0; i < 14; i++) fprintf(stderr, " %lld", t[34 + i] - t[0]);
      fprintf(stderr, "\n   stage seen full by the MMA thread:  ");
      for(int i = 0; i < 14; i++) fprintf(stderr, " %lld", t[48 + i] - t[0]);
      fprintf(stderr, "\n   GEMM 1 issuer: total %lld cycles, blocked on stage %lld, drain %lld | GEMM 2 issuer: total %lld, blocked on transforms %lld, matrix buffer %lld | epilogue warp 0 / 15 blocked on rest accumulators %lld / %lld, on matrices %lld / %lld\n",
              t[69] - t[0], t[64], t[67], t[68] - t[0], t[65], t[66], t[70], t[72], t[71], t[73]);
    }
  }
  return SMPLPP_OK;
}
}
```

### smplpp_b200/csrc/tc3_layout.cuh

```cuda
#pragma once
#include <cuda_fp16.h>

#include "common.cuh"
#include "skin_common.cuh"

namespace tc3
{
using namespace sb;
constexpr int MV = 128;
constexpr int NF = 96;
constexpr int ROWB = 64;
constexpr int KP = kBlendK;
constexpr int KUSED = kPoseDim + kShapeDim;
constexpr int NKB = KP * 2 / ROWB;
constexpr int A_PART = 3 * MV * ROWB;
constexpr int B_PART = NF * ROWB;
constexpr int STAGE = 2 * A_PART + 2 * B_PART;
constexpr int SUBF = 8;
constexpr int SUBN = SUBF * kXformFloats;
constexpr int KJ = skin::KJ;
constexpr int G_PART = SUBN * ROWB;
constexpr int G_STAGE = 2 * G_PART;
constexpr int NSUB = NF / SUBF;
constexpr int EPI_WARPS = 16;
constexpr int EPI_FR = 2;
constexpr int FR_WARP = NSUB * EPI_FR;
constexpr int CTRL_WARPS = 4;
constexpr int THREADS = 32 * (CTRL_WARPS + EPI_WARPS);
constexpr int STG_FLOATS = EPI_FR * 32 * 3;
constexpr int STG_BYTES = EPI_WARPS * STG_FLOATS * 4;
template<int ST, int GS, int EPI>
struct Layout
{
  static constexpr int OFF_G = ST * STAGE;
  static constexpr int OFF_STG = OFF_G + GS * G_STAGE;
  static constexpr int OFF_BAR = OFF_STG + (EPI == 0 ? STG_BYTES : 0);
  static constexpr int SMEM_BYTES = 1024 + OFF_BAR + 512;
  static_assert(OFF_STG % 1024 == 0, "swizzle atoms stay aligned");
  static_assert(SMEM_BYTES <= 227 * 1024, "shared memory budget");
};
constexpr int TMEM_COLS = 512;
constexpr int COL_M = 3 * NF;
constexpr int COL_W = COL_M + 2 * SUBN;
constexpr int TRIPLES = NKB * 6;
constexpr int COEF_EXP = 6, W_EXP = skin::W_EXP, G_EXP = skin::G_EXP;
static_assert(COL_W + 2 * (KJ / 2) == TMEM_COLS, "TMEM column map");
static_assert(STAGE % 1024 == 0 && G_STAGE % 1024 == 0, "swizzle atoms stay aligned");

__host__ __device__ constexpr int coef_row(int n)
{
  return ((n % SUBF) / EPI_FR) * FR_WARP + (n / SUBF) * EPI_FR + (n % EPI_FR);
}


__host__ __device__ constexpr uint32_t swz64(uint32_t o)
{
  return o ^ (((o >> 7) & 3u) << 4);
}

__device__ __forceinline__ void split8_store(const float (&x)[8], uint8_t * hi_dst, uint8_t * lo_dst)
{
  uint32_t h[4], l[4];
#pragma unroll
  for(int i = 0; i < 4; i++)
  {
    const float a = x[2 * i], b = x[2 * i + 1];
    const float ah = __half2float(__float2half_rn(a)), bh = __half2float(__float2half_rn(b));
    h[i] = skin::pack_half2(ah, bh);
    l[i] = skin::pack_half2(a - ah, b - bh);
  }
  *reinterpret_cast<uint4 *>(hi_dst) = make_uint4(h[0], h[1], h[2], h[3]);
  *reinterpret_cast<uint4 *>(lo_dst) = make_uint4(l[0], l[1], l[2], l[3]);
}

inline size_t img_g_offset(int Bpad)
{
  return align_up(static_cast<size_t>(2) * Bpad * KP * sizeof(__half));
}
}
```

### smplpp_b200/csrc/tc_ptx.cuh

```cuda
#pragma once
#include <cuda_runtime.h>

#include <cstdint>

namespace sb
{
namespace ptx
{
__device__ __forceinline__ uint32_t smem_u32(const void * p)
{
  return static_cast<uint32_t>(__cvta_generic_to_shared(p));
}

__device__ __forceinline__ bool elect_one()
{
  uint32_t pred = 0;
  asm volatile(
      "{\n\t"
      ".reg .pred P;\n\t"
      "elect.sync _|P, 0xffffffff;\n\t"
      "selp.u32 %0, 1, 0, P;\n\t"
      "}\n"
      : "=r"(pred));
  return pred != 0;
}

__device__ __forceinline__ float4 lds128(uint32_t addr)
{
  float4 v;
  asm volatile("ld.shared.v4.f32 {%0, %1, %2, %3}, [%4];" : "=f"(v.x), "=f"(v.y), "=f"(v.z), "=f"(v.w) : "r"(addr));
  return v;
}
__device__ __forceinline__ float2 lds64(uint32_t addr)
{
  float2 v;
  asm volatile("ld.shared.v2.f32 {%0, %1}, [%2];" : "=f"(v.x), "=f"(v.y) : "r"(addr));
  return v;
}
__device__ __forceinline__ void sts32(uint32_t addr, float v)
{
  asm volatile("st.shared.f32 [%0], %1;" ::"r"(addr), "f"(v) : "memory");
}

__device__ __forceinline__ void sts64(uint32_t addr, float2 v)
{
  asm volatile("st.shared.v2.f32 [%0], {%1, %2};" ::"r"(addr), "f"(v.x), "f"(v.y) : "memory");
}
__device__ __forceinline__ void sts128(uint32_t addr, float4 v)
{
  asm volatile("st.shared.v4.f32 [%0], {%1, %2, %3, %4};" ::"r"(addr), "f"(v.x), "f"(v.y), "f"(v.z), "f"(v.w) : "memory");
}
__device__ __forceinline__ float lds32(uint32_t addr)
{
  float v;
  asm volatile("ld.shared.f32 %0, [%1];" : "=f"(v) : "r"(addr));
  return v;
}

__device__ __forceinline__ void mbar_init(uint64_t * bar, uint32_t count)
{
  asm volatile("mbarrier.init.shared::cta.b64 [%0], %1;" ::"r"(smem_u32(bar)), "r"(count) : "memory");
}
__device__ __forceinline__ void fence_barrier_init()
{
  asm volatile("fence.mbarrier_init.release.cluster;" ::: "memory");
}
__device__ __forceinline__ void fence_proxy_async()
{
  asm volatile("fence.proxy.async.shared::cta;" ::: "memory");
}
__device__ __forceinline__ void mbar_expect_tx(uint64_t * bar, uint32_t bytes)
{
  asm volatile("mbarrier.arrive.expect_tx.shared::cta.b64 _, [%0], %1;" ::"r"(smem_u32(bar)), "r"(bytes) : "memory");
}
__device__ __forceinline__ void mbar_arrive(uint64_t * bar)
{
  asm volatile("mbarrier.arrive.shared::cta.b64 _, [%0];" ::"r"(smem_u32(bar)) : "memory");
}
__device__ __forceinline__ bool mbar_try_wait(uint64_t * bar, uint32_t parity)
{
  uint32_t ok;
  asm volatile(
      "{\n\t"
      ".reg .pred P;\n\t"
      "mbarrier.try_wait.parity.shared::cta.b64 P, [%1], %2;\n\t"
      "selp.u32 %0, 1, 0, P;\n\t"
      "}\n"
      : "=r"(ok)
      : "r"(smem_u32(bar)), "r"(parity)
      : "memory");
  return ok != 0;
}
__device__ __forceinline__ bool mbar_test_wait(uint64_t * bar, uint32_t parity)
{
  uint32_t ok;
  asm volatile(
      "{\n\t"
      ".reg .pred P;\n\t"
      "mbarrier.test_wait.parity.shared::cta.b64 P, [%1], %2;\n\t"
      "selp.u32 %0, 1, 0, P;\n\t"
      "}\n"
      : "=r"(ok)
      : "r"(smem_u32(bar)), "r"(parity)
      : "memory");
  return ok != 0;
}
__device__ __forceinline__ void mbar_wait(uint64_t * bar, uint32_t parity)
{
  uint32_t spins = 0;
  while(!mbar_try_wait(bar, parity))
  {
    if(++spins > (1u << 26)) __trap();
  }
}

__device__ __forceinline__ void mbar_wait_a(uint32_t bar, uint32_t parity)
{
  uint32_t spins = 0, ok;
  do
  {
    asm volatile(
        "{\n\t"
        ".reg .pred P;\n\t"
        "mbarrier.try_wait.parity.shared::cta.b64 P, [%1], %2;\n\t"
        "selp.u32 %0, 1, 0, P;\n\t"
        "}\n"
        : "=r"(ok)
        : "r"(bar), "r"(parity)
        : "memory");
    if(!ok && ++spins > (1u << 26)) __trap();
  } while(!ok);
}
__device__ __forceinline__ void mbar_arrive_a(uint32_t bar)
{
  asm volatile("mbarrier.arrive.shared::cta.b64 _, [%0];" ::"r"(bar) : "memory");
}
__device__ __forceinline__ void mbar_expect_tx_a(uint32_t bar, uint32_t bytes)
{
  asm volatile("mbarrier.arrive.expect_tx.shared::cta.b64 _, [%0], %1;" ::"r"(bar), "r"(bytes) : "memory");
}
__device__ __forceinline__ void bulk_load_1d_a(uint32_t smem_dst, const void * gmem_src, uint32_t bytes, uint32_t bar)
{
  asm volatile("cp.async.bulk.shared::cluster.global.mbarrier::complete_tx::bytes [%0], [%1], %2, [%3];"
               :
               : "r"(smem_dst), "l"(reinterpret_cast<uint64_t>(gmem_src)), "r"(bytes), "r"(bar)
               : "memory");
}
__device__ __forceinline__ void tc_commit_a(uint32_t bar)
{
  asm volatile("tcgen05.commit.cta_group::1.mbarrier::arrive::one.shared::cluster.b64 [%0];" ::"r"(bar) : "memory");
}

__device__ __forceinline__ void prefetch_tensormap(const void * tmap)
{
  asm volatile("prefetch.tensormap [%0];" ::"l"(reinterpret_cast<uint64_t>(tmap)) : "memory");
}
__device__ __forceinline__ void tma_load_2d(void * smem_dst, const void * tmap, int c0, int c1, uint64_t * bar)
{
  asm volatile("cp.async.bulk.tensor.2d.shared::cluster.global.tile.mbarrier::complete_tx::bytes [%0], [%1, {%3, %4}], [%2];"
               :
               : "r"(smem_u32(smem_dst)), "l"(reinterpret_cast<uint64_t>(tmap)), "r"(smem_u32(bar)), "r"(c0), "r"(c1)
               : "memory");
}
__device__ __forceinline__ void bulk_load_1d(void * smem_dst, const void * gmem_src, uint32_t bytes, uint64_t * bar)
{
  asm volatile("cp.async.bulk.shared::cluster.global.mbarrier::complete_tx::bytes [%0], [%1], %2, [%3];"
               :
               : "r"(smem_u32(smem_dst)), "l"(reinterpret_cast<uint64_t>(gmem_src)), "r"(bytes), "r"(smem_u32(bar))
               : "memory");
}

__device__ __forceinline__ void bulk_store_1d(void * gmem_dst, uint32_t smem_src, uint32_t bytes)
{
  asm volatile("cp.async.bulk.global.shared::cta.bulk_group [%0], [%1], %2;"
               :
               : "l"(reinterpret_cast<uint64_t>(gmem_dst)), "r"(smem_src), "r"(bytes)
               : "memory");
}
__device__ __forceinline__ void bulk_commit()
{
  asm volatile("cp.async.bulk.commit_group;" ::: "memory");
}
template<int kPending>
__device__ __forceinline__ void bulk_wait_read()
{
  asm volatile("cp.async.bulk.wait_group.read %0;" ::"n"(kPending) : "memory");
}

template<int kCols>
__device__ __forceinline__ void tmem_alloc(uint32_t * smem_result)
{
  asm volatile("tcgen05.alloc.cta_group::1.sync.aligned.shared::cta.b32 [%0], %1;" ::"r"(smem_u32(smem_result)), "n"(kCols)
               : "memory");
  asm volatile("tcgen05.relinquish_alloc_permit.cta_group::1.sync.aligned;" ::: "memory");
}
template<int kCols>
__device__ __forceinline__ void tmem_dealloc(uint32_t taddr)
{
  asm volatile("tcgen05.dealloc.cta_group::1.sync.aligned.b32 %0, %1;" ::"r"(taddr), "n"(kCols) : "memory");
}
__device__ __forceinline__ void tc_fence_before()
{
  asm volatile("tcgen05.fence::before_thread_sync;" ::: "memory");
}
__device__ __forceinline__ void tc_fence_after()
{
  asm volatile("tcgen05.fence::after_thread_sync;" ::: "memory");
}
__device__ __forceinline__ void tc_commit(uint64_t * bar)
{
  asm volatile("tcgen05.commit.cta_group::1.mbarrier::arrive::one.shared::cluster.b64 [%0];" ::"r"(smem_u32(bar)) : "memory");
}

template<bool kTf32>
__device__ __forceinline__ void umma(uint32_t d_tmem, uint64_t a_desc, uint64_t b_desc, uint32_t idesc, uint32_t accumulate)
{
  if constexpr(kTf32)
  {
    asm volatile(
        "{\n\t"
        ".reg .pred p;\n\t"
        "setp.ne.b32 p, %4, 0;\n\t"
        "tcgen05.mma.cta_group::1.kind::tf32 [%0], %1, %2, %3, p;\n\t"
        "}\n" ::"r"(d_tmem),
        "l"(a_desc), "l"(b_desc), "r"(idesc), "r"(accumulate)
        : "memory");
  }
  else
  {
    asm volatile(
        "{\n\t"
        ".reg .pred p;\n\t"
        "setp.ne.b32 p, %4, 0;\n\t"
        "tcgen05.mma.cta_group::1.kind::f16 [%0], %1, %2, %3, p;\n\t"
        "}\n" ::"r"(d_tmem),
        "l"(a_desc), "l"(b_desc), "r"(idesc), "r"(accumulate)
        : "memory");
  }
}

__device__ __forceinline__ void tmem_ld_x8(uint32_t taddr, float (&v)[8])
{
  uint32_t r[8];
  asm volatile("tcgen05.ld.sync.aligned.32x32b.x8.b32 {%0, %1, %2, %3, %4, %5, %6, %7}, [%8];"
               : "=r"(r[0]), "=r"(r[1]), "=r"(r[2]), "=r"(r[3]), "=r"(r[4]), "=r"(r[5]), "=r"(r[6]), "=r"(r[7])
               : "r"(taddr));
#pragma unroll
  for(int i = 0; i < 8; i++) v[i] = __uint_as_float(r[i]);
}
__device__ __forceinline__ void tmem_ld_x2(uint32_t taddr, float (&v)[2])
{
  uint32_t r[2];
  asm volatile("tcgen05.ld.sync.aligned.32x32b.x2.b32 {%0, %1}, [%2];" : "=r"(r[0]), "=r"(r[1]) : "r"(taddr));
  v[0] = __uint_as_float(r[0]), v[1] = __uint_as_float(r[1]);
}
__device__ __forceinline__ void tmem_ld_x8p(uint32_t taddr, float * v)
{
  uint32_t r[8];
  asm volatile("tcgen05.ld.sync.aligned.32x32b.x8.b32 {%0, %1, %2, %3, %4, %5, %6, %7}, [%8];"
               : "=r"(r[0]), "=r"(r[1]), "=r"(r[2]), "=r"(r[3]), "=r"(r[4]), "=r"(r[5]), "=r"(r[6]), "=r"(r[7])
               : "r"(taddr));
#pragma unroll
  for(int i = 0; i < 8; i++) v[i] = __uint_as_float(r[i]);
}
__device__ __forceinline__ void tmem_ld_x4(uint32_t taddr, float (&v)[4])
{
  uint32_t r[4];
  asm volatile("tcgen05.ld.sync.aligned.32x32b.x4.b32 {%0, %1, %2, %3}, [%4];"
               : "=r"(r[0]), "=r"(r[1]), "=r"(r[2]), "=r"(r[3])
               : "r"(taddr));
#pragma unroll
  for(int i = 0; i < 4; i++) v[i] = __uint_as_float(r[i]);
}
__device__ __forceinline__ void tmem_ld_x16(uint32_t taddr, float * v)
{
  uint32_t r[16];
  asm volatile(
      "tcgen05.ld.sync.aligned.32x32b.x16.b32 {%0, %1, %2, %3, %4, %5, %6, %7, %8, %9, %10, %11, %12, %13, %14, %15}, [%16];"
      : "=r"(r[0]), "=r"(r[1]), "=r"(r[2]), "=r"(r[3]), "=r"(r[4]), "=r"(r[5]), "=r"(r[6]), "=r"(r[7]), "=r"(r[8]),
        "=r"(r[9]), "=r"(r[10]), "=r"(r[11]), "=r"(r[12]), "=r"(r[13]), "=r"(r[14]), "=r"(r[15])
      : "r"(taddr));
#pragma unroll
  for(int i = 0; i < 16; i++) v[i] = __uint_as_float(r[i]);
}
__device__ __forceinline__ void tmem_st_x16(uint32_t taddr, const uint32_t (&r)[16])
{
  asm volatile(
      "tcgen05.st.sync.aligned.32x32b.x16.b32 [%0], {%1, %2, %3, %4, %5, %6, %7, %8, %9, %10, %11, %12, %13, %14, %15, %16};"
      :
      : "r"(taddr), "r"(r[0]), "r"(r[1]), "r"(r[2]), "r"(r[3]), "r"(r[4]), "r"(r[5]), "r"(r[6]), "r"(r[7]), "r"(r[8]),
        "r"(r[9]), "r"(r[10]), "r"(r[11]), "r"(r[12]), "r"(r[13]), "r"(r[14]), "r"(r[15])
      : "memory");
}
__device__ __forceinline__ void tmem_st_wait()
{
  asm volatile("tcgen05.wait::st.sync.aligned;" ::: "memory");
}
__device__ __forceinline__ void umma_f16_ts(uint32_t d_tmem, uint32_t a_tmem, uint64_t b_desc, uint32_t idesc, uint32_t accumulate)
{
  asm volatile(
      "{\n\t"
      ".reg .pred p;\n\t"
      "setp.ne.b32 p, %4, 0;\n\t"
      "tcgen05.mma.cta_group::1.kind::f16 [%0], [%1], %2, %3, p;\n\t"
      "}\n" ::"r"(d_tmem),
      "r"(a_tmem), "l"(b_desc), "r"(idesc), "r"(accumulate)
      : "memory");
}
__device__ __forceinline__ void umma_f16_ss(uint32_t d_tmem, uint64_t a_desc, uint64_t b_desc, uint32_t idesc, uint32_t accumulate)
{
  asm volatile(
      "{\n\t"
      ".reg .pred p;\n\t"
      "setp.ne.b32 p, %4, 0;\n\t"
      "tcgen05.mma.cta_group::1.kind::f16 [%0], %1, %2, %3, p;\n\t"
      "}\n" ::"r"(d_tmem),
      "l"(a_desc), "l"(b_desc), "r"(idesc), "r"(accumulate)
      : "memory");
}
template<int kRowBytes>
__host__ __device__ constexpr uint32_t smem_desc_hi()
{
  static_assert(kRowBytes == 64 || kRowBytes == 128, "row = one swizzle span");
  return static_cast<uint32_t>((8 * kRowBytes) >> 4) | (1u << 14) | ((kRowBytes == 128 ? 2u : 4u) << 29);
}
__device__ __forceinline__ void umma_f16_ss_lo(uint32_t d_tmem, uint32_t a_lo, uint32_t b_lo, uint32_t desc_hi, uint32_t idesc,
                                               uint32_t accumulate)
{
  asm volatile(
      "{\n\t"
      ".reg .pred p;\n\t"
      ".reg .b64 da, db;\n\t"
      "setp.ne.b32 p, %5, 0;\n\t"
      "mov.b64 da, {%1, %3};\n\t"
      "mov.b64 db, {%2, %3};\n\t"
      "tcgen05.mma.cta_group::1.kind::f16 [%0], da, db, %4, p;\n\t"
      "}\n" ::"r"(d_tmem),
      "r"(a_lo), "r"(b_lo), "r"(desc_hi), "r"(idesc), "r"(accumulate)
      : "memory");
}
__device__ __forceinline__ void umma_f16_ts_lo(uint32_t d_tmem, uint32_t a_tmem, uint32_t b_lo, uint32_t desc_hi, uint32_t idesc,
                                               uint32_t accumulate)
{
  asm volatile(
      "{\n\t"
      ".reg .pred p;\n\t"
      ".reg .b64 db;\n\t"
      "setp.ne.b32 p, %5, 0;\n\t"
      "mov.b64 db, {%2, %3};\n\t"
      "tcgen05.mma.cta_group::1.kind::f16 [%0], [%1], db, %4, p;\n\t"
      "}\n" ::"r"(d_tmem),
      "r"(a_tmem), "r"(b_lo), "r"(desc_hi), "r"(idesc), "r"(accumulate)
      : "memory");
}
__host__ __device__ constexpr uint32_t make_idesc_f16(int m, int n)
{
  return (1u << 4) | (static_cast<uint32_t>(n >> 3) << 17) | (static_cast<uint32_t>(m >> 4) << 24);
}
__device__ __forceinline__ void tmem_ld_wait()
{
  asm volatile("tcgen05.wait::ld.sync.aligned;" ::: "memory");
}

__host__ __device__ constexpr uint32_t make_idesc(bool tf32, int m, int n)
{
  return (1u << 4) | ((tf32 ? 2u : 1u) << 7) | ((tf32 ? 2u : 1u) << 10) | (static_cast<uint32_t>(n >> 3) << 17)
         | (static_cast<uint32_t>(m >> 4) << 24);
}

template<int kRowBytes>
__device__ __forceinline__ uint64_t make_smem_desc(uint32_t smem_addr)
{
  static_assert(kRowBytes == 64 || kRowBytes == 128, "row = one swizzle span");
  constexpr uint64_t layout = kRowBytes == 128 ? 2 : 4;
  constexpr uint64_t sbo = (8 * kRowBytes) >> 4;
  return static_cast<uint64_t>((smem_addr & 0x3FFFF) >> 4) | (sbo << 32) | (1ull << 46) | (layout << 61);
}
}
}
```

Before: 20.90 million.

## Run blend-skin tensor-core kernel as 2-CTA cluster pairs with paired UMMA

Converts the tc3 blend/skin kernel to launch in clusters of two CTAs that use cta_group::2 tcgen05 MMAs (M=256) with a paired TMEM allocation. Each CTA now loads only its half of the coefficient (B) and transform (G) operands, and the coefficient/transform image layout is re-laid into half blocks to match. Barriers are replicated across the pair through cluster-mapped arrivals. The aim is to halve per-CTA shared memory traffic and staging for the shared operand, which frees space for a third pipeline stage. The cost is cluster synchronization overhead and more intricate barrier logic that could deadlock or mis-order if any count is wrong.

```diff
diff --git a/smplpp_b200/csrc/common.cuh b/smplpp_b200/csrc/common.cuh
--- a/smplpp_b200/csrc/common.cuh
+++ b/smplpp_b200/csrc/common.cuh
@@ -101,7 +101,7 @@
   bool tc2_ready = false;
   void * basis_img16 = nullptr;
   bool tc3_ready = false;
-  int sm_count = 0;
+  int tc3_clusters = 0;
 };
 }
 
diff --git a/smplpp_b200/csrc/forward.cu b/smplpp_b200/csrc/forward.cu
--- a/smplpp_b200/csrc/forward.cu
+++ b/smplpp_b200/csrc/forward.cu
@@ -53,22 +53,16 @@
   {
     if(img_b && b < Bpad)
     {
-      const long long fb = b / tc3::NF;
-      const int nf = static_cast<int>(b - fb * tc3::NF);
       const uint4 z = make_uint4(0u, 0u, 0u, 0u);
       if(lane < tc3::KP / 8)
       {
-        uint8_t * blk = img_b + (static_cast<size_t>(fb) * tc3::NKB + lane / 4) * (2 * tc3::B_PART);
-        const uint32_t o = static_cast<uint32_t>(tc3::coef_row(nf) * tc3::ROWB + (lane % 4) * 16);
-        *reinterpret_cast<uint4 *>(blk + tc3::swz64(o)) = z;
-        *reinterpret_cast<uint4 *>(blk + tc3::swz64(tc3::B_PART + o)) = z;
-      }
-      uint8_t * blk = img_g + (static_cast<size_t>(fb) * tc3::NSUB + nf / tc3::SUBF) * tc3::G_STAGE;
+        *reinterpret_cast<uint4 *>(img_b + tc3::coef_img_off(b, lane, 0)) = z;
+        *reinterpret_cast<uint4 *>(img_b + tc3::coef_img_off(b, lane, 1)) = z;
+      }
       for(int c = lane; c < kXformFloats * 4; c += 32)
       {
-        const uint32_t o = static_cast<uint32_t>(((nf % tc3::SUBF) * kXformFloats + c / 4) * tc3::ROWB + (c % 4) * 16);
-        *reinterpret_cast<uint4 *>(blk + tc3::swz64(o)) = z;
-        *reinterpret_cast<uint4 *>(blk + tc3::swz64(tc3::G_PART + o)) = z;
+        *reinterpret_cast<uint4 *>(img_g + tc3::xform_img_off(b, c / 4, c % 4, 0)) = z;
+        *reinterpret_cast<uint4 *>(img_g + tc3::xform_img_off(b, c / 4, c % 4, 1)) = z;
       }
     }
     return;
@@ -165,9 +159,6 @@
       for(int e = 0; e < 12; e++) sG[warp][lane][e] = G[e];
     }
     __syncwarp();
-    const long long fb = b / tc3::NF;
-    const int nf = static_cast<int>(b - fb * tc3::NF);
-    uint8_t * blk = img_g + (static_cast<size_t>(fb) * tc3::NSUB + nf / tc3::SUBF) * tc3::G_STAGE;
     for(int c = lane; c < kXformFloats * 4; c += 32)
     {
       const int e = c / 4, cj = c % 4;
@@ -178,8 +169,7 @@
         const int j = cj * 8 + jj;
         x[jj] = j < kJoints ? sG[warp][j][e] * static_cast<float>(1 << tc3::G_EXP) : 0.f;
       }
-      const uint32_t o = static_cast<uint32_t>(((nf % tc3::SUBF) * kXformFloats + e) * tc3::ROWB + cj * 16);
-      tc3::split8_store(x, blk + tc3::swz64(o), blk + tc3::swz64(tc3::G_PART + o));
+      tc3::split8_store(x, img_g + tc3::xform_img_off(b, e, cj, 0), img_g + tc3::xform_img_off(b, e, cj, 1));
     }
   }
   if(coef)
@@ -199,11 +189,7 @@
       float x[8];
 #pragma unroll
       for(int e = 0; e < 8; e++) x[e] = lane * 8 + e < tc3::KUSED ? sC[warp][lane * 8 + e] * static_cast<float>(1 << tc3::COEF_EXP) : 0.f;
-      const long long fb = b / tc3::NF;
-      const int r = tc3::coef_row(static_cast<int>(b - fb * tc3::NF));
-      uint8_t * blk = img_b + (static_cast<size_t>(fb) * tc3::NKB + lane / 4) * (2 * tc3::B_PART);
-      const uint32_t o = static_cast<uint32_t>(r * tc3::ROWB + (lane % 4) * 16);
-      tc3::split8_store(x, blk + tc3::swz64(o), blk + tc3::swz64(tc3::B_PART + o));
+      tc3::split8_store(x, img_b + tc3::coef_img_off(b, lane, 0), img_b + tc3::coef_img_off(b, lane, 1));
     }
   }
 }
diff --git a/smplpp_b200/csrc/skin_tc3.cu b/smplpp_b200/csrc/skin_tc3.cu
--- a/smplpp_b200/csrc/skin_tc3.cu
+++ b/smplpp_b200/csrc/skin_tc3.cu
@@ -73,11 +73,7 @@
     }
 #pragma unroll
     for(int e = 0; e < 8; e++) x[e] = (f < B && ck * 8 + e < tc3::KUSED) ? x[e] * static_cast<float>(1 << tc3::COEF_EXP) : 0.f;
-    const long long fb = f / tc3::NF;
-    const int r = tc3::coef_row(static_cast<int>(f - fb * tc3::NF));
-    uint8_t * blk = img_b + (static_cast<size_t>(fb) * tc3::NKB + ck / 4) * (2 * tc3::B_PART);
-    const uint32_t o = static_cast<uint32_t>(r * tc3::ROWB + (ck % 4) * 16);
-    tc3::split8_store(x, blk + tc3::swz64(o), blk + tc3::swz64(tc3::B_PART + o));
+    tc3::split8_store(x, img_b + tc3::coef_img_off(f, ck, 0), img_b + tc3::coef_img_off(f, ck, 1));
   }
   else if(i < n_coef + n_xf)
   {
@@ -92,21 +88,15 @@
       const int j = cj * 8 + jj;
       x[jj] = (f < B && j < kJoints) ? __ldg(xforms + (f * kJoints + j) * kXformFloats + e) * static_cast<float>(1 << tc3::G_EXP) : 0.f;
     }
-    const long long fb = f / tc3::NF;
-    const int nf = static_cast<int>(f - fb * tc3::NF);
-    uint8_t * blk = img_g + (static_cast<size_t>(fb) * tc3::NSUB + nf / tc3::SUBF) * tc3::G_STAGE;
-    const uint32_t o = static_cast<uint32_t>(((nf % tc3::SUBF) * kXformFloats + e) * tc3::ROWB + cj * 16);
-    tc3::split8_store(x, blk + tc3::swz64(o), blk + tc3::swz64(tc3::G_PART + o));
-  }
-}
-
-template<int STAGES, int GSLOTS, int EPI, bool DBG = false>
+    tc3::split8_store(x, img_g + tc3::xform_img_off(f, e, cj, 0), img_g + tc3::xform_img_off(f, e, cj, 1));
+  }
+}
+
+template<bool DBG = false>
 __global__ void __launch_bounds__(tc3::THREADS, 1)
     blend_skin_tc3_kernel(const tc3::Params p)
 {
   using namespace tc3;
-  using L = Layout<STAGES, GSLOTS, EPI>;
-  constexpr int OFF_G = L::OFF_G, OFF_STG = L::OFF_STG, OFF_BAR = L::OFF_BAR;
   extern __shared__ uint8_t smem_raw[];
   uint8_t * smem = reinterpret_cast<uint8_t *>((reinterpret_cast<uintptr_t>(smem_raw) + 1023) & ~uintptr_t(1023));
   uint64_t * bars = reinterpret_cast<uint64_t *>(smem + OFF_BAR);
@@ -122,37 +112,43 @@
   uint64_t * rest_free = p_full + 1;
   uint64_t * w_ready = rest_free + 1;
   uint32_t * tmem_slot = reinterpret_cast<uint32_t *>(w_ready + 1);
+  const uint32_t a_full = bar32;
+  const uint32_t a_empty = a_full + 8 * STAGES, a_gfull = a_empty + 8 * STAGES, a_gempty = a_gfull + 8 * GSLOTS,
+                 a_mfull = a_gempty + 8 * GSLOTS, a_mempty = a_mfull + 16, a_pfull = a_mempty + 16, a_rest = a_pfull + 8,
+                 a_wready = a_rest + 8;
 
   const int warp = threadIdx.x >> 5, lane = threadIdx.x & 31;
-  const int it0 = static_cast<int>(static_cast<long long>(blockIdx.x) * p.nitems / gridDim.x);
-  const int it1 = static_cast<int>(static_cast<long long>(blockIdx.x + 1) * p.nitems / gridDim.x);
+  const uint32_t rank = ptx::cluster_ctarank();
+  const int pair = static_cast<int>(blockIdx.x >> 1), npairs = static_cast<int>(gridDim.x >> 1);
+  const int it0 = static_cast<int>(static_cast<long long>(pair) * p.nitems / npairs);
+  const int it1 = static_cast<int>(static_cast<long long>(pair + 1) * p.nitems / npairs);
   const int nit = it1 - it0;
 
   if(warp == 0 && lane == 0)
   {
     for(int s = 0; s < STAGES; s++)
     {
-      ptx::mbar_init(&full[s], 1);
+      ptx::mbar_init(&full[s], rank == 0 ? 2 : 1);
       ptx::mbar_init(&empty[s], 1);
     }
     for(int s = 0; s < GSLOTS; s++)
     {
-      ptx::mbar_init(&g_full[s], 1);
+      ptx::mbar_init(&g_full[s], rank == 0 ? 2 : 1);
       ptx::mbar_init(&g_empty[s], 1);
     }
     for(int i = 0; i < 2; i++)
     {
       ptx::mbar_init(&m_full[i], 1);
-      ptx::mbar_init(&m_empty[i], EPI_WARPS);
+      ptx::mbar_init(&m_empty[i], 2 * EPI_WARPS);
     }
     ptx::mbar_init(p_full, 1);
-    ptx::mbar_init(rest_free, EPI_WARPS);
-    ptx::mbar_init(w_ready, 4);
+    ptx::mbar_init(rest_free, 2 * EPI_WARPS);
+    ptx::mbar_init(w_ready, 8);
     ptx::fence_barrier_init();
   }
-  if(warp == 1) ptx::tmem_alloc<TMEM_COLS>(tmem_slot);
+  if(warp == 1) ptx::tmem_alloc_pair<TMEM_COLS>(tmem_slot);
   ptx::tc_fence_before();
-  __syncthreads();
+  ptx::cluster_sync();
   ptx::tc_fence_after();
   const uint32_t tmem_base = *tmem_slot;
   long long * dbg = (DBG && p.dbg) ? p.dbg + static_cast<size_t>(blockIdx.x) * 256 : nullptr;
@@ -163,87 +159,101 @@
   if(warp < CTRL_WARPS)
   {
   asm volatile("setmaxnreg.dec.sync.aligned.u32 32;");
+  const int total_kb = TC3_OFF(32) ? 0 : nit * NKB;
+  const int total_g = TC3_OFF(64) ? 0 : nit * NSUB;
   if(warp == 0)
   {
     if(ptx::elect_one())
     {
-      const int total_kb = TC3_OFF(32) ? 0 : nit * NKB;
-      int kb = 0, tile = it0 / p.nfb, fb = it0 % p.nfb;
+      int kb = 0, tp = it0 / p.nfb, fb = it0 % p.nfb;
       for(int kbn = 0; kbn < total_kb; kbn++)
       {
         const uint32_t s = static_cast<uint32_t>(kbn % STAGES);
-        const uint8_t * srca = p.img_a + (static_cast<size_t>(tile) * NKB + kb) * (2 * A_PART);
-        const uint8_t * srcb = p.img_b + (static_cast<size_t>(fb) * NKB + kb) * (2 * B_PART);
-        const uint32_t dst = smem32 + s * STAGE, fbar = bar32 + 8 * s;
-        ptx::mbar_wait_a(bar32 + 8 * (STAGES + s), ((kbn / STAGES) & 1) ^ 1);
+        const uint8_t * srca = p.img_a + (static_cast<size_t>(2 * tp + rank) * NKB + kb) * (2 * A_PART);
+        const uint8_t * srcb = p.img_b + ((static_cast<size_t>(fb) * NKB + kb) * 2 + rank) * H_COPY;
+        const uint32_t dst = smem32 + s * STAGE, fbar = a_full + 8 * s;
+        ptx::mbar_wait_a(a_empty + 8 * s, ((kbn / STAGES) & 1) ^ 1);
         ptx::mbar_expect_tx_a(fbar, STAGE);
         ptx::bulk_load_1d_a(dst, srca, 2 * A_PART, fbar);
-        ptx::bulk_load_1d_a(dst + 2 * A_PART, srcb, 2 * B_PART, fbar);
+        ptx::bulk_load_1d_a(dst + 2 * A_PART, srcb, H_COPY, fbar);
         if(dbg && kbn < 14) dbg[34 + kbn] = clock64();
         if(++kb == NKB)
         {
           kb = 0;
-          if(++fb == p.nfb) fb = 0, tile++;
-        }
-      }
+          if(++fb == p.nfb) fb = 0, tp++;
+        }
+      }
+      for(int kbn = total_kb; kbn < total_kb + STAGES; kbn++) ptx::mbar_wait_a(a_empty + 8 * (kbn % STAGES), ((kbn / STAGES) & 1) ^ 1);
     }
   }
   else if(warp == 2)
   {
     if(ptx::elect_one())
     {
-      const int total_g = TC3_OFF(64) ? 0 : nit * NSUB;
       int sb = 0, fb = it0 % p.nfb;
       for(int gn = 0; gn < total_g; gn++)
       {
         const uint32_t s = static_cast<uint32_t>(gn % GSLOTS);
-        const uint8_t * src = p.img_g + (static_cast<size_t>(fb) * NSUB + sb) * G_STAGE;
-        const uint32_t fbar = bar32 + 8 * (2 * STAGES + s);
-        ptx::mbar_wait_a(bar32 + 8 * (2 * STAGES + GSLOTS + s), ((gn / GSLOTS) & 1) ^ 1);
-        ptx::mbar_expect_tx_a(fbar, G_STAGE);
-        ptx::bulk_load_1d_a(smem32 + OFF_G + s * G_STAGE, src, G_STAGE, fbar);
+        const uint8_t * src = p.img_g + ((static_cast<size_t>(fb) * NSUB + sb) * 2 + rank) * H_COPY;
+        const uint32_t fbar = a_gfull + 8 * s;
+        ptx::mbar_wait_a(a_gempty + 8 * s, ((gn / GSLOTS) & 1) ^ 1);
+        ptx::mbar_expect_tx_a(fbar, H_COPY);
+        ptx::bulk_load_1d_a(smem32 + OFF_G + s * H_COPY, src, H_COPY, fbar);
         if(++sb == NSUB)
         {
           sb = 0;
           if(++fb == p.nfb) fb = 0;
         }
       }
+      for(int gn = total_g; gn < total_g + GSLOTS; gn++) ptx::mbar_wait_a(a_gempty + 8 * (gn % GSLOTS), ((gn / GSLOTS) & 1) ^ 1);
+    }
+  }
+  else if(rank != 0)
+  {
+    if(ptx::elect_one())
+    {
+      const bool stages = warp == 3;
+      const int total = stages ? total_kb : total_g, ring = stages ? STAGES : GSLOTS;
+      const uint32_t local = stages ? a_full : a_gfull, remote = ptx::mapa(local, 0);
+      for(int n = 0; n < total; n++)
+      {
+        const uint32_t s = static_cast<uint32_t>(n % ring);
+        ptx::mbar_wait_a(local + 8 * s, (n / ring) & 1);
+        ptx::mbar_arrive_cluster(remote + 8 * s);
+      }
     }
   }
   else if(warp == 1 || warp == 3)
   {
     if(ptx::elect_one())
     {
-      constexpr uint32_t idesc1 = ptx::make_idesc_f16(MV, NF);
-      constexpr uint32_t idesc2 = ptx::make_idesc_f16(MV, SUBN);
+      constexpr uint32_t idesc1 = ptx::make_idesc_f16(2 * MV, NF);
+      constexpr uint32_t idesc2 = ptx::make_idesc_f16(2 * MV, SUBN);
       static_assert(NSUB % GSLOTS == 0 && ((NSUB / GSLOTS) & 1) == 0, "transform ring: slot and parity of a sub-batch do not depend on the item");
       static_assert((NSUB & 3) == 0, "matrix buffers: parity of a sub-batch does not depend on the item");
       constexpr uint32_t DHI = ptx::smem_desc_hi<ROWB>();
       const uint32_t smem16 = smem32 >> 4;
-      const uint32_t a_full = bar32;
-      const uint32_t a_empty = a_full + 8 * STAGES, a_gfull = a_empty + 8 * STAGES, a_gempty = a_gfull + 8 * GSLOTS,
-                     a_mfull = a_gempty + 8 * GSLOTS, a_mempty = a_mfull + 16, a_pfull = a_mempty + 16, a_rest = a_pfull + 8,
-                     a_wready = a_rest + 8;
       auto g1_mma = [&](uint32_t st16, int hpar, int i, uint32_t acc) {
         const int t = i / 3, c = i % 3;
         const int a_part = hpar == 0 ? (t == 2 ? 1 : 0) : (t == 0 ? 1 : 0);
         const int b_part = hpar == 0 ? 0 : (t == 0 ? 0 : 1);
         const int ks = hpar == 0 ? (t == 1 ? 1 : 0) : (t == 1 ? 0 : 1);
-        ptx::umma_f16_ss_lo(tmem_base + c * NF, st16 + ((a_part * A_PART + c * MV * ROWB + ks * 32) >> 4),
-                            st16 + ((2 * A_PART + b_part * B_PART + ks * 32) >> 4), DHI, idesc1, acc);
+        ptx::umma_f16_ss_lo_pair(tmem_base + c * NF, st16 + ((a_part * A_PART + c * MV * ROWB + ks * 32) >> 4),
+                                 st16 + ((2 * A_PART + b_part * H_PART + ks * 32) >> 4), DHI, idesc1, acc);
       };
       auto g2_mma = [&](uint32_t dm, uint32_t aw, uint32_t sg16, int j) {
         const int prod = j >> 1, ks = j & 1;
         const int pa = prod == 1 ? 1 : 0, pb = prod == 2 ? 1 : 0;
-        ptx::umma_f16_ts_lo(dm, aw + pa * (KJ / 2) + ks * 8, sg16 + ((pb * G_PART + ks * 32) >> 4), DHI, idesc2, j != 0 ? 1u : 0u);
+        ptx::umma_f16_ts_lo_pair(dm, aw + pa * (KJ / 2) + ks * 8, sg16 + ((pb * H_PART + ks * 32) >> 4), DHI, idesc2, j != 0 ? 1u : 0u);
       };
-      auto g1_half = [&](int h, int kbn0) {
-        const int kbn = kbn0 + (h >> 1);
-        const uint32_t s = static_cast<uint32_t>(kbn % STAGES);
+      uint32_t s1 = 0, ph1 = 0;
+      int kbn = 0;
+      auto g1_half = [&](int h) {
+        const uint32_t s = s1;
         const uint32_t st16 = smem16 + s * (STAGE >> 4);
         if((h & 1) == 0)
         {
-          if(!TC3_OFF(32)) TC3_TIMED(w_stage, ptx::mbar_wait_a(a_full + 8 * s, (kbn / STAGES) & 1));
+          if(!TC3_OFF(32)) TC3_TIMED(w_stage, ptx::mbar_wait_a(a_full + 8 * s, ph1));
           ptx::tc_fence_after();
           if(dbg && kbn < 14) dbg[48 + kbn] = clock64();
 #pragma unroll
@@ -255,15 +265,17 @@
 #pragma unroll
           for(int i = 0; i < 9; i++)
             if(!DBG || !(p.dbg_mode & 8)) g1_mma(st16, 1, i, 1u);
-          if(!TC3_OFF(32)) ptx::tc_commit_a(a_empty + 8 * s);
+          if(!TC3_OFF(32)) ptx::tc_commit_pair_a(a_empty + 8 * s);
+          if(++s1 == STAGES) s1 = 0, ph1 ^= 1;
+          if(dbg) kbn++;
         }
       };
       if(dbg) dbg[0] = clock64();
       if(nit > 0 && warp == 3)
       {
 #pragma unroll
-        for(int h = 0; h < 2 * NKB; h++) g1_half(h, 0);
-        if(!TC3_OFF(512)) ptx::tc_commit_a(a_pfull);
+        for(int h = 0; h < 2 * NKB; h++) g1_half(h);
+        if(!TC3_OFF(512)) ptx::tc_commit_pair_a(a_pfull);
       }
       if(dbg) dbg[1] = clock64();
       if(warp == 3)
@@ -273,22 +285,21 @@
           if(!TC3_OFF(512)) TC3_TIMED(w_rest, ptx::mbar_wait_a(a_rest, k & 1));
           ptx::tc_fence_after();
 #pragma unroll
-          for(int h = 0; h < 2 * NKB; h++) g1_half(h, (k + 1) * NKB);
-          if(!TC3_OFF(512)) ptx::tc_commit_a(a_pfull);
+          for(int h = 0; h < 2 * NKB; h++) g1_half(h);
+          if(!TC3_OFF(512)) ptx::tc_commit_pair_a(a_pfull);
         }
         if(dbg) dbg[64] = w_stage, dbg[67] = w_rest, dbg[69] = clock64();
       }
-      int wcount = 0, prev_tile = -1;
+      int wcount = 0, fb = it0 % p.nfb;
       for(int k = 0; k < (warp == 3 ? 0 : nit); k++)
       {
-        const int tile = (it0 + k) / p.nfb;
-        if(tile != prev_tile)
+        if(k == 0 || fb == 0)
         {
           ptx::mbar_wait_a(a_wready, wcount & 1);
           ptx::tc_fence_after();
           wcount++;
-          prev_tile = tile;
-        }
+        }
+        if(++fb == p.nfb) fb = 0;
         const uint32_t aw = tmem_base + COL_W;
 #pragma unroll
         for(int sb = 0; sb < NSUB; sb++)
@@ -297,13 +308,13 @@
           if(!TC3_OFF(64)) TC3_TIMED(w_gfull, ptx::mbar_wait_a(a_gfull + 8 * gs, (sb / GSLOTS) & 1));
           if(!TC3_OFF(256)) TC3_TIMED(w_mempty, ptx::mbar_wait_a(a_mempty + 8 * b, ((sb >> 1) & 1) ^ 1));
           ptx::tc_fence_after();
-          const uint32_t sg16 = smem16 + ((OFF_G + gs * G_STAGE) >> 4);
+          const uint32_t sg16 = smem16 + ((OFF_G + gs * H_COPY) >> 4);
           const uint32_t dm = tmem_base + COL_M + b * SUBN;
 #pragma unroll
           for(int j = 0; j < 6; j++)
             if(!DBG || !(p.dbg_mode & 4)) g2_mma(dm, aw, sg16, j);
-          if(!TC3_OFF(256)) ptx::tc_commit_a(a_mfull + 8 * b);
-          if(!TC3_OFF(64)) ptx::tc_commit_a(a_gempty + 8 * gs);
+          if(!TC3_OFF(256)) ptx::tc_commit_pair_a(a_mfull + 8 * b);
+          if(!TC3_OFF(64)) ptx::tc_commit_pair_a(a_gempty + 8 * gs);
         }
         if(dbg && k < 30) dbg[2 + k] = clock64();
       }
@@ -318,10 +329,8 @@
     const int q = warp & 3;
     const int fp = ew >> 2;
     const uint32_t lane_taddr = tmem_base + (static_cast<uint32_t>(q * 32) << 16);
-    const uint32_t my_stg = ptx::smem_u32(smem + OFF_STG) + ew * STG_FLOATS * 4;
     const float sp = p.scale_p;
-    const uint32_t a_mfull = bar32 + 16 * (STAGES + GSLOTS);
-    const uint32_t a_mempty = a_mfull + 16, a_pfull = a_mempty + 16, a_rest = a_pfull + 8, a_wready = a_rest + 8;
+    const uint32_t c_mempty = ptx::mapa(a_mempty, 0), c_rest = ptx::mapa(a_rest, 0), c_wready = ptx::mapa(a_wready, 0);
     const unsigned fstride = static_cast<unsigned>(p.V) * 3u;
     int prev_tile = -1;
     int wv0 = 0, nvalid = 0;
@@ -330,7 +339,8 @@
     for(int k = 0; k < nit; k++)
     {
       const int item = it0 + k;
-      const int tile = item / p.nfb, f0 = (item - tile * p.nfb) * NF;
+      const int tp = item / p.nfb, f0 = (item - tp * p.nfb) * NF;
+      const int tile = 2 * tp + static_cast<int>(rank);
       if(tile != prev_tile)
       {
         prev_tile = tile;
@@ -343,11 +353,11 @@
           ptx::tmem_st_wait();
           ptx::tc_fence_before();
           __syncwarp();
-          if(lane == 0) ptx::mbar_arrive_a(a_wready);
+          if(lane == 0) ptx::mbar_arrive_cluster(c_wready);
         }
         sm = p.scale_m / p.wsum[vc];
-        const float * tp = p.basis + static_cast<size_t>(3) * vc * kBlendK + KUSED;
-        T0 = __ldg(tp) * sm, T1 = __ldg(tp + kBlendK) * sm, T2 = __ldg(tp + 2 * kBlendK) * sm;
+        const float * tq = p.basis + static_cast<size_t>(3) * vc * kBlendK + KUSED;
+        T0 = __ldg(tq) * sm, T1 = __ldg(tq + kBlendK) * sm, T2 = __ldg(tq + 2 * kBlendK) * sm;
       }
       float trx = 0.f, try_ = 0.f, trz = 0.f;
       if(lane < FR_WARP)
@@ -374,7 +384,7 @@
       ptx::tmem_ld_wait();
       ptx::tc_fence_before();
       __syncwarp();
-      if(lane == 0 && !TC3_OFF(512)) ptx::mbar_arrive_a(a_rest);
+      if(lane == 0 && !TC3_OFF(512)) ptx::mbar_arrive_cluster(c_rest);
       {
         const float s = sp * sm;
 #pragma unroll
@@ -385,8 +395,7 @@
           R[2][i] = fmaf(R[2][i], s, T2);
         }
       }
-      float * outp = p.out + (static_cast<size_t>(f0 + fp * EPI_FR) * p.V + wv0) * 3;
-      float * outl = outp + lane * 3;
+      float * outl = p.out + (static_cast<size_t>(f0 + fp * EPI_FR) * p.V + wv0 + lane) * 3;
       const int nfv = lane < nvalid ? p.B - f0 - fp * EPI_FR : 0;
 #pragma unroll
       for(int sb = 0; sb < NSUB; sb++)
@@ -417,7 +426,7 @@
         ptx::tmem_ld_wait();
         ptx::tc_fence_before();
         __syncwarp();
-        if(lane == 0 && !TC3_OFF(256)) ptx::mbar_arrive_a(a_mempty + 8 * h);
+        if(lane == 0 && !TC3_OFF(256)) ptx::mbar_arrive_cluster(c_mempty + 8 * h);
         if(TC3_OFF(128)) continue;
 #pragma unroll
         for(int t = 0; t < EPI_FR; t++)
@@ -427,38 +436,14 @@
           const float ox = fmaf(m[0], rx, fmaf(m[1], ry, fmaf(m[2], rz, fmaf(m[3], sm, tr[t][0]))));
           const float oy = fmaf(m[4], rx, fmaf(m[5], ry, fmaf(m[6], rz, fmaf(m[7], sm, tr[t][1]))));
           const float oz = fmaf(m[8], rx, fmaf(m[9], ry, fmaf(m[10], rz, fmaf(m[11], sm, tr[t][2]))));
-          if constexpr(EPI == 0)
+          float * o = outl + static_cast<size_t>((sb * SUBF + t) * fstride);
+          if(sb * SUBF + t < nfv && (!DBG || !(p.dbg_mode & 2) || ox == 1.2345e30f))
           {
-            const uint32_t sa = my_stg + (t * 96 + lane * 3) * 4;
-            ptx::sts32(sa, ox);
-            ptx::sts32(sa + 4, oy);
-            ptx::sts32(sa + 8, oz);
+            __stcs(o, ox);
+            __stcs(o + 1, oy);
+            __stcs(o + 2, oz);
           }
-          else
-          {
-            float * o = outl + static_cast<size_t>((sb * SUBF + t) * fstride);
-            if(sb * SUBF + t < nfv && (!DBG || !(p.dbg_mode & 2) || ox == 1.2345e30f))
-            {
-              __stcs(o, ox);
-              __stcs(o + 1, oy);
-              __stcs(o + 2, oz);
-            }
-          }
-        }
-        if constexpr(EPI != 0) continue;
-        __syncwarp();
-#pragma unroll
-        for(int i = 0; i < EPI_FR * 48 / 32; i++)
-        {
-          const int idx = 32 * i + lane;
-          const int t = idx / 48;
-          const int w2 = idx - 48 * t;
-          const int f = f0 + sb * SUBF + fp * EPI_FR + t;
-          const float2 val = ptx::lds64(my_stg + idx * 8);
-          if(f < p.B && 2 * w2 < 3 * nvalid)
-            __stcs(reinterpret_cast<float2 *>(outp + (static_cast<size_t>(sb * SUBF + t) * p.V) * 3) + w2, val);
-        }
-        __syncwarp();
+        }
       }
     }
     if(dbg && (ew == 0 || ew == 15) && lane == 0)
@@ -470,8 +455,9 @@
 #undef TC3_TIMED
 #undef TC3_OFF
   ptx::tc_fence_before();
-  __syncthreads();
-  if(warp == 1) ptx::tmem_dealloc<TMEM_COLS>(tmem_base);
+  __syncwarp();
+  ptx::cluster_sync();
+  if(warp == 1) ptx::tmem_dealloc_pair<TMEM_COLS>(tmem_base);
 }
 
 namespace sb
@@ -482,24 +468,34 @@
   return align_up(2 * bpad * tc3::KP * sizeof(__half)) + align_up(2 * bpad * kXformFloats * tc3::KJ * sizeof(__half));
 }
 
+static int tc3_tiles(const ModelDev & d)
+{
+  return (d.tc2_tiles + 1) & ~1;
+}
+
 int tc3_prepare_model(ModelDev & d)
 {
   d.tc3_ready = false;
   if(!d.tc2_ready) return SMPLPP_OK;
-  const long long n = static_cast<long long>(d.tc2_tiles) * 3 * tc3::MV * tc3::KP;
+  const long long n = static_cast<long long>(tc3_tiles(d)) * 3 * tc3::MV * tc3::KP;
   SB_CUDA(cudaMalloc(&d.basis_img16, static_cast<size_t>(2) * n * sizeof(__half)));
-  basis_image_f16_kernel<<<static_cast<unsigned>((n + 255) / 256), 256>>>(d.basis, d.V, d.tc2_tiles, ldexpf(1.f, d.tc2_basis_exp),
+  basis_image_f16_kernel<<<static_cast<unsigned>((n + 255) / 256), 256>>>(d.basis, d.V, tc3_tiles(d), ldexpf(1.f, d.tc2_basis_exp),
                                                                          static_cast<uint8_t *>(d.basis_img16));
   SB_LAUNCHED();
   SB_CUDA(cudaDeviceSynchronize());
-  SB_CUDA(cudaFuncSetAttribute(blend_skin_tc3_kernel<2, 6, 1>, cudaFuncAttributeMaxDynamicSharedMemorySize, tc3::Layout<2, 6, 1>::SMEM_BYTES));
-  SB_CUDA(cudaFuncSetAttribute(blend_skin_tc3_kernel<2, 6, 1, true>, cudaFuncAttributeMaxDynamicSharedMemorySize, tc3::Layout<2, 6, 1>::SMEM_BYTES));
-  SB_CUDA(cudaFuncSetAttribute(blend_skin_tc3_kernel<3, 3, 1>, cudaFuncAttributeMaxDynamicSharedMemorySize, tc3::Layout<3, 3, 1>::SMEM_BYTES));
-  SB_CUDA(cudaFuncSetAttribute(blend_skin_tc3_kernel<2, 6, 0>, cudaFuncAttributeMaxDynamicSharedMemorySize, tc3::Layout<2, 6, 0>::SMEM_BYTES));
-  int dev = 0;
-  SB_CUDA(cudaGetDevice(&dev));
-  SB_CUDA(cudaDeviceGetAttribute(&d.sm_count, cudaDevAttrMultiProcessorCount, dev));
-  d.tc3_ready = d.sm_count > 0;
+  SB_CUDA(cudaFuncSetAttribute(blend_skin_tc3_kernel<false>, cudaFuncAttributeMaxDynamicSharedMemorySize, tc3::SMEM_BYTES));
+  SB_CUDA(cudaFuncSetAttribute(blend_skin_tc3_kernel<true>, cudaFuncAttributeMaxDynamicSharedMemorySize, tc3::SMEM_BYTES));
+  cudaLaunchConfig_t cfg = {};
+  cudaLaunchAttribute attr[1];
+  attr[0].id = cudaLaunchAttributeClusterDimension;
+  attr[0].val.clusterDim.x = 2, attr[0].val.clusterDim.y = 1, attr[0].val.clusterDim.z = 1;
+  cfg.gridDim = dim3(2);
+  cfg.blockDim = dim3(tc3::THREADS);
+  cfg.dynamicSmemBytes = tc3::SMEM_BYTES;
+  cfg.attrs = attr;
+  cfg.numAttrs = 1;
+  SB_CUDA(cudaOccupancyMaxActiveClusters(&d.tc3_clusters, blend_skin_tc3_kernel<false>, &cfg));
+  d.tc3_ready = d.tc3_clusters > 0;
   return SMPLPP_OK;
 }
 
@@ -529,9 +525,9 @@
   p.V = d.V;
   p.B = B;
   p.Bpad = Bpad;
-  p.ntiles = d.tc2_tiles;
+  p.ntiles = tc3_tiles(d);
   p.nfb = Bpad / tc3::NF;
-  p.nitems = p.ntiles * p.nfb;
+  p.nitems = p.ntiles / 2 * p.nfb;
   p.scale_p = ldexpf(1.f, -(d.tc2_basis_exp + tc3::COEF_EXP));
   p.scale_m = ldexpf(1.f, -(tc3::W_EXP + tc3::G_EXP));
   p.img_a = static_cast<const uint8_t *>(d.basis_img16);
@@ -542,10 +538,9 @@
   p.wsum = d.lbs_wsum;
   p.theta = theta;
   p.out = out;
-  int grid = p.nitems < d.sm_count ? p.nitems : d.sm_count;
+  int grid = 2 * (p.nitems < d.tc3_clusters ? p.nitems : d.tc3_clusters);
   static const int grid_env = getenv("SMPLPP_TC3_GRID") ? atoi(getenv("SMPLPP_TC3_GRID")) : 0;
-  static const int ring_env = getenv("SMPLPP_TC3_RING") ? atoi(getenv("SMPLPP_TC3_RING")) : 0;
-  if(grid_env > 0 && grid_env < grid) grid = grid_env;
+  if(grid_env > 0 && grid_env < grid) grid = grid_env < 2 ? 2 : grid_env & ~1;
   static const bool dbg_on = getenv("SMPLPP_TC3_DBG") != nullptr;
   p.dbg = nullptr;
   p.dbg_mode = dbg_on ? atoi(getenv("SMPLPP_TC3_DBG")) >> 1 : 0;
@@ -554,14 +549,20 @@
     SB_CUDA(cudaMalloc(&p.dbg, static_cast<size_t>(grid) * 256 * sizeof(long long)));
     SB_CUDA(cudaMemsetAsync(p.dbg, 0, static_cast<size_t>(grid) * 256 * sizeof(long long), st));
   }
-  if(ring_env == 1)
-    blend_skin_tc3_kernel<3, 3, 1><<<grid, tc3::THREADS, tc3::Layout<3, 3, 1>::SMEM_BYTES, st>>>(p);
-  else if(ring_env == 2)
-    blend_skin_tc3_kernel<2, 6, 0><<<grid, tc3::THREADS, tc3::Layout<2, 6, 0>::SMEM_BYTES, st>>>(p);
-  else if(dbg_on)
-    blend_skin_tc3_kernel<2, 6, 1, true><<<grid, tc3::THREADS, tc3::Layout<2, 6, 1>::SMEM_BYTES, st>>>(p);
+  cudaLaunchConfig_t cfg = {};
+  cudaLaunchAttribute attr[1];
+  attr[0].id = cudaLaunchAttributeClusterDimension;
+  attr[0].val.clusterDim.x = 2, attr[0].val.clusterDim.y = 1, attr[0].val.clusterDim.z = 1;
+  cfg.gridDim = dim3(static_cast<unsigned>(grid));
+  cfg.blockDim = dim3(tc3::THREADS);
+  cfg.dynamicSmemBytes = tc3::SMEM_BYTES;
+  cfg.stream = st;
+  cfg.attrs = attr;
+  cfg.numAttrs = 1;
+  if(dbg_on)
+    SB_CUDA(cudaLaunchKernelEx(&cfg, blend_skin_tc3_kernel<true>, p));
   else
-    blend_skin_tc3_kernel<2, 6, 1><<<grid, tc3::THREADS, tc3::Layout<2, 6, 1>::SMEM_BYTES, st>>>(p);
+    SB_CUDA(cudaLaunchKernelEx(&cfg, blend_skin_tc3_kernel<false>, p));
   SB_LAUNCHED();
   if(dbg_on)
   {
@@ -569,9 +570,15 @@
     std::vector<long long> h(static_cast<size_t>(grid) * 256);
     SB_CUDA(cudaMemcpy(h.data(), p.dbg, h.size() * sizeof(long long), cudaMemcpyDeviceToHost));
     cudaFree(p.dbg);
-    for(int cta : {0, grid / 2})
+    for(int cta : {0, grid / 2 & ~1, grid / 2 | 1})
     {
       const long long * t = h.data() + static_cast<size_t>(cta) * 256;
+      if(cta & 1)
+      {
+        fprintf(stderr, "[tc3 dbg] cta %d (odd): epilogue %lld .. %lld | epilogue warp 0 / 15 blocked on rest accumulators %lld / %lld, on matrices %lld / %lld\n",
+                cta, t[32] - t[32], t[33] - t[32], t[70], t[72], t[71], t[73]);
+        continue;
+      }
       fprintf(stderr, "[tc3 dbg] cta %d: first GEMM 1 issued +%lld | items", cta, t[1] - t[0]);
       for(int k = 0; k < 30 && t[2 + k]; k++) fprintf(stderr, " %lld", t[2 + k] - (k ? t[1 + k] : t[1]));
       fprintf(stderr, " | epilogue %lld .. %lld\n", t[32] - t[0], t[33] - t[0]);
diff --git a/smplpp_b200/csrc/tc3_layout.cuh b/smplpp_b200/csrc/tc3_layout.cuh
--- a/smplpp_b200/csrc/tc3_layout.cuh
+++ b/smplpp_b200/csrc/tc3_layout.cuh
@@ -9,43 +9,36 @@
 using namespace sb;
 constexpr int MV = 128;
 constexpr int NF = 96;
+constexpr int NH = NF / 2;
 constexpr int ROWB = 64;
 constexpr int KP = kBlendK;
 constexpr int KUSED = kPoseDim + kShapeDim;
 constexpr int NKB = KP * 2 / ROWB;
 constexpr int A_PART = 3 * MV * ROWB;
-constexpr int B_PART = NF * ROWB;
-constexpr int STAGE = 2 * A_PART + 2 * B_PART;
+constexpr int H_PART = NH * ROWB;
+constexpr int H_COPY = 2 * H_PART;
+constexpr int STAGE = 2 * A_PART + H_COPY;
 constexpr int SUBF = 8;
 constexpr int SUBN = SUBF * kXformFloats;
 constexpr int KJ = skin::KJ;
-constexpr int G_PART = SUBN * ROWB;
-constexpr int G_STAGE = 2 * G_PART;
 constexpr int NSUB = NF / SUBF;
 constexpr int EPI_WARPS = 16;
 constexpr int EPI_FR = 2;
 constexpr int FR_WARP = NSUB * EPI_FR;
 constexpr int CTRL_WARPS = 4;
 constexpr int THREADS = 32 * (CTRL_WARPS + EPI_WARPS);
-constexpr int STG_FLOATS = EPI_FR * 32 * 3;
-constexpr int STG_BYTES = EPI_WARPS * STG_FLOATS * 4;
-template<int ST, int GS, int EPI>
-struct Layout
-{
-  static constexpr int OFF_G = ST * STAGE;
-  static constexpr int OFF_STG = OFF_G + GS * G_STAGE;
-  static constexpr int OFF_BAR = OFF_STG + (EPI == 0 ? STG_BYTES : 0);
-  static constexpr int SMEM_BYTES = 1024 + OFF_BAR + 512;
-  static_assert(OFF_STG % 1024 == 0, "swizzle atoms stay aligned");
-  static_assert(SMEM_BYTES <= 227 * 1024, "shared memory budget");
-};
+constexpr int STAGES = 3;
+constexpr int GSLOTS = 6;
+constexpr int OFF_G = STAGES * STAGE;
+constexpr int OFF_BAR = OFF_G + GSLOTS * H_COPY;
+constexpr int SMEM_BYTES = 1024 + OFF_BAR + 512;
+static_assert(SMEM_BYTES <= 227 * 1024, "shared memory budget");
 constexpr int TMEM_COLS = 512;
 constexpr int COL_M = 3 * NF;
 constexpr int COL_W = COL_M + 2 * SUBN;
-constexpr int TRIPLES = NKB * 6;
 constexpr int COEF_EXP = 6, W_EXP = skin::W_EXP, G_EXP = skin::G_EXP;
 static_assert(COL_W + 2 * (KJ / 2) == TMEM_COLS, "TMEM column map");
-static_assert(STAGE % 1024 == 0 && G_STAGE % 1024 == 0, "swizzle atoms stay aligned");
+static_assert(STAGE % 1024 == 0 && H_PART % 1024 == 0, "swizzle atoms stay aligned");
 
 __host__ __device__ constexpr int coef_row(int n)
 {
@@ -56,6 +49,22 @@
 __host__ __device__ constexpr uint32_t swz64(uint32_t o)
 {
   return o ^ (((o >> 7) & 3u) << 4);
+}
+
+__host__ __device__ constexpr uint32_t half_block_off(int r, int c, int part)
+{
+  return swz64(static_cast<uint32_t>((r / NH) * H_COPY + part * H_PART + (r % NH) * ROWB + c * 16));
+}
+__host__ __device__ inline size_t coef_img_off(long long f, int ck, int part)
+{
+  const long long fb = f / NF;
+  return (static_cast<size_t>(fb) * NKB + ck / 4) * (2 * H_COPY) + half_block_off(coef_row(static_cast<int>(f - fb * NF)), ck % 4, part);
+}
+__host__ __device__ inline size_t xform_img_off(long long f, int e, int cj, int part)
+{
+  const long long fb = f / NF;
+  const int nf = static_cast<int>(f - fb * NF);
+  return (static_cast<size_t>(fb) * NSUB + nf / SUBF) * (2 * H_COPY) + half_block_off((nf % SUBF) * kXformFloats + e, cj, part);
 }
 
 __device__ __forceinline__ void split8_store(const float (&x)[8], uint8_t * hi_dst, uint8_t * lo_dst)
diff --git a/smplpp_b200/csrc/tc_ptx.cuh b/smplpp_b200/csrc/tc_ptx.cuh
--- a/smplpp_b200/csrc/tc_ptx.cuh
+++ b/smplpp_b200/csrc/tc_ptx.cuh
@@ -149,6 +149,74 @@
 __device__ __forceinline__ void tc_commit_a(uint32_t bar)
 {
   asm volatile("tcgen05.commit.cta_group::1.mbarrier::arrive::one.shared::cluster.b64 [%0];" ::"r"(bar) : "memory");
+}
+
+__device__ __forceinline__ uint32_t cluster_ctarank()
+{
+  uint32_t r;
+  asm volatile("mov.u32 %0, %%cluster_ctarank;" : "=r"(r));
+  return r;
+}
+__device__ __forceinline__ void cluster_sync()
+{
+  asm volatile("barrier.cluster.arrive.release.aligned;\n\tbarrier.cluster.wait.acquire.aligned;" ::: "memory");
+}
+__device__ __forceinline__ uint32_t mapa(uint32_t addr, uint32_t rank)
+{
+  uint32_t r;
+  asm volatile("mapa.shared::cluster.u32 %0, %1, %2;" : "=r"(r) : "r"(addr), "r"(rank));
+  return r;
+}
+__device__ __forceinline__ void mbar_arrive_cluster(uint32_t cbar)
+{
+  asm volatile("mbarrier.arrive.shared::cluster.b64 _, [%0];" ::"r"(cbar) : "memory");
+}
+__device__ __forceinline__ void tc_commit_pair_a(uint32_t bar)
+{
+  asm volatile("tcgen05.commit.cta_group::2.mbarrier::arrive::one.shared::cluster.multicast::cluster.b64 [%0], %1;" ::"r"(bar),
+               "h"(static_cast<uint16_t>(0x3))
+               : "memory");
+}
+template<int kCols>
+__device__ __forceinline__ void tmem_alloc_pair(uint32_t * smem_result)
+{
+  asm volatile("tcgen05.alloc.cta_group::2.sync.aligned.shared::cta.b32 [%0], %1;" ::"r"(smem_u32(smem_result)), "n"(kCols)
+               : "memory");
+  asm volatile("tcgen05.relinquish_alloc_permit.cta_group::2.sync.aligned;" ::: "memory");
+}
+template<int kCols>
+__device__ __forceinline__ void tmem_dealloc_pair(uint32_t taddr)
+{
+  asm volatile("tcgen05.dealloc.cta_group::2.sync.aligned.b32 %0, %1;" ::"r"(taddr), "n"(kCols) : "memory");
+}
+__device__ __forceinline__ void umma_f16_ss_lo_pair(uint32_t d_tmem, uint32_t a_lo, uint32_t b_lo, uint32_t desc_hi, uint32_t idesc,
+                                                    uint32_t accumulate)
+{
+  asm volatile(
+      "{\n\t"
+      ".reg .pred p;\n\t"
+      ".reg .b64 da, db;\n\t"
+      "setp.ne.b32 p, %5, 0;\n\t"
+      "mov.b64 da, {%1, %3};\n\t"
+      "mov.b64 db, {%2, %3};\n\t"
+      "tcgen05.mma.cta_group::2.kind::f16 [%0], da, db, %4, p;\n\t"
+      "}\n" ::"r"(d_tmem),
+      "r"(a_lo), "r"(b_lo), "r"(desc_hi), "r"(idesc), "r"(accumulate)
+      : "memory");
+}
+__device__ __forceinline__ void umma_f16_ts_lo_pair(uint32_t d_tmem, uint32_t a_tmem, uint32_t b_lo, uint32_t desc_hi, uint32_t idesc,
+                                                    uint32_t accumulate)
+{
+  asm volatile(
+      "{\n\t"
+      ".reg .pred p;\n\t"
+      ".reg .b64 db;\n\t"
+      "setp.ne.b32 p, %5, 0;\n\t"
+      "mov.b64 db, {%2, %3};\n\t"
+      "tcgen05.mma.cta_group::2.kind::f16 [%0], [%1], db, %4, p;\n\t"
+      "}\n" ::"r"(d_tmem),
+      "r"(a_tmem), "r"(b_lo), "r"(desc_hi), "r"(idesc), "r"(accumulate)
+      : "memory");
 }
 
 __device__ __forceinline__ void prefetch_tensormap(const void * tmap)
```

Measured after the change: 20.35 million (median of 6 runs). -2.6%, worse.
